# Geo3DSmart/PDANet

Measured on AMD Instinct MI355X. Metric: scenes/sec (16384-pt ONCE, PDA-SSD forward+backward), higher is better.
Workload: dtype f32; 1 GPU; once16k_b2_detector_fwd_bwd_adam; scenes_per_gpu=2, global_batch=2, parallelism=dp1, world_size_seen=1, cpu_affinity=GPU-local NUMA node of 0000:5d:00.0: 128 CPUs, full=False, graph_tail=False, graph_head=True

## Files before the change

include/pda_train.h:

```cpp
#ifndef PDA_TRAIN_H
#define PDA_TRAIN_H
#include "pda_pointnet2.h"

#ifdef __cplusplus
extern "C" {
#endif

int pda_grad_norm(const float *g, int64_t n, float *norm_out, float *scratch1024, pda_stream_t stream);
int pda_adam_onecycle_step(float *p, const float *g, float *m, float *v, int64_t n, float lr,
                           float beta1, float beta2, float eps, float wd, int step,
                           const float *total_norm, float max_norm, pda_stream_t stream);

int64_t pda_bn_relu_scratch_bytes(int c);
int pda_bn_relu_fwd(const float *x, const float *gamma, const float *beta, float *running_mean,
                    float *running_var, float *y, float *mean_invstd, void *scratch, int64_t rows, int c,
                    float eps, float momentum, pda_stream_t stream);
int pda_bn_relu_bwd(const float *x, const float *grad_y, const float *gamma, const float *beta,
                    const float *mean_invstd, float *grad_x, float *grad_gamma, float *grad_beta,
                    void *scratch, int64_t rows, int c, pda_stream_t stream);
int pda_bn_relu_fwd_counted(const float *x, const float *gamma, const float *beta, float *running_mean, float *running_var,
                            float *y, float *mean_invstd, void *scratch, int64_t rows, int c, float eps, float momentum,
                            const int32_t *count, int32_t *status, int relu, int training, pda_stream_t stream);
int pda_bn_relu_bwd_counted(const float *x, const float *grad_y, const float *gamma, const float *beta,
                            const float *mean_invstd, float *grad_x, float *grad_gamma, float *grad_beta, void *scratch,
// ... 38 lines not shown
                             float *grad_gamma, float *grad_beta, void *scratch, int64_t rows, int d,
                             pda_stream_t stream);

int64_t pda_linear_wgrad_scratch_bytes(int64_t tokens, int in_features, int out_features);
int pda_linear_wgrad_form(int64_t tokens, int in_features, int out_features);
int pda_linear_wgrad(const float *x, const float *grad_out, float *grad_weight, float *grad_bias,
                     void *scratch, int64_t tokens, int in_features, int out_features, pda_stream_t stream);
int pda_linear_wgrad_bn(const float *x, const float *grad_out, float *grad_weight, float *grad_bias, void *scratch,
                        int64_t tokens, int in_features, int out_features, const float *x_mean_invstd,
                        const float *x_gamma, const float *x_beta, pda_stream_t stream);

typedef struct pda_param_grad_entry {
    int32_t kind, count;
    const float *part, *part_bias;
    float *dst, *dst_bias;
    int64_t nm;
    int32_t n, cols;
    int64_t ld;
} pda_param_grad_entry_t;
int pda_linear_wgrad_partials(const float *x, const float *grad_out, void *scratch, int want_bias, int64_t tokens,
                              int in_features, int out_features, int *slices, pda_stream_t stream);
int pda_linear_wgrad_bn_partials(const float *x, const float *grad_out, void *scratch, int64_t tokens, int in_features,
                                 int out_features, const float *x_mean_invstd, const float *x_gamma,
                                 const float *x_beta, int *slices, pda_stream_t stream);
int pda_layer_norm_bwd_partials(const float *x, const float *grad_y, const void *grad_y2, int grad_y2_is_bf16,
                                const float *gamma, const float *mean_rstd, float *grad_x, uint16_t *grad_x_bf16,
                                void *scratch, int64_t rows, int d, int *nblocks, pda_stream_t stream);
int pda_param_grad_reduce_grouped(const pda_param_grad_entry_t *entries, int n, pda_stream_t stream);

int64_t pda_gemm_split_bn_tiles(int64_t tokens);
int pda_gemm_split_bn(const float *x, const void *wf, float *y, int64_t tokens, int k, int n_out,
                      const float *in_mean_invstd, const float *in_gamma, const float *in_beta, int stats_mode,
                      double *partial, pda_stream_t stream);
int pda_gemm_split_maxpool(const float *x, const void *wf, const float *bias, float *out, int64_t tokens, int k, int n_out,
                           int ns, int relu, pda_stream_t stream);
int pda_gemm_split_gather(const float *point_rows, const float *xyz, const float *new_xyz, const int32_t *idx,
                          const float *w1, int ldw1, const float *bias1, const void *wf, const float *bias2, float *y,
                          int b, int n, int m, int ns, int k, int n_out, int relu, pda_stream_t stream);
int pda_bn_stats_fwd(const float *x, float *running_mean, float *running_var, float *mean_invstd, void *scratch,
                     int64_t rows, int c, float eps, float momentum, pda_stream_t stream);
int pda_bn_finalize_fwd(const double *partial, int nblocks, int c, int64_t count, float eps, float momentum,
                        float *mean_invstd, float *running_mean, float *running_var, pda_stream_t stream);
int pda_bn_relu_max_pool_apply(const float *x, const float *gamma, const float *beta, const float *mean_invstd,
                               float *out, uint8_t *arg, int64_t groups, int ns, int c, pda_stream_t stream);

int64_t pda_colsum_scratch_bytes(int cols);
int pda_colsum_bf16(const uint16_t *g, float *out, void *scratch, int64_t rows, int cols, pda_stream_t stream);

int pda_assemble_tokens(const float *rppe, const float *dscale, const float *feats, const int32_t *idx,
                        const float *glob, float *out, int b, int n, int m, int nsample, int c,
                        pda_stream_t stream);
int pda_assemble_tokens_grad(const float *grad_out, const float *dscale, const float *feats, const int32_t *idx,
                             float *grad_rppe, float *grad_dscale, float *grad_feats, float *grad_glob,
                             int b, int n, int m, int nsample, int c, pda_stream_t stream);

int pda_add_max_pool(const float *a, const float *b, float *out, uint8_t *arg, int64_t groups, int seq, int d,
                     pda_stream_t stream);
int pda_max_pool_scatter(const float *grad_out, const uint8_t *arg, float *grad_x, int64_t groups, int seq,
                         int d, pda_stream_t stream);
int pda_add_max_pool_bf16(const float *a, const uint16_t *b, float *out, uint8_t *arg, int64_t groups, int seq,
                          int d, pda_stream_t stream);
int pda_max_pool_scatter_bf16(const float *grad_out, const uint8_t *arg, float *grad_x, uint16_t *grad_x_bf16,
                              int64_t groups, int seq, int d, pda_stream_t stream);

int pda_bn_relu_fwd_weighted(const float *x, const float *gamma, const float *beta, float *running_mean,
                             float *running_var, float *y, float *mean_invstd, void *scratch, int64_t rows, int c,
                             float eps, float momentum, const float *row_weight, int64_t count, pda_stream_t stream);
int pda_bn_relu_bwd_weighted(const float *x, const float *grad_y, const float *gamma, const float *beta,
                             const float *mean_invstd, float *grad_x, float *grad_gamma, float *grad_beta,
                             void *scratch, int64_t rows, int c, const float *row_weight, int64_t count,
                             pda_stream_t stream);

int pda_ragged_plan(const int32_t *idx, int32_t *cnt, int32_t *off, int32_t *rowmap, float *row_weight, int64_t groups,
                    int nsample, pda_stream_t stream);
int pda_assemble_tokens_ragged(const float *rppe, const float *dscale, const float *feats, const int32_t *idx,
                               const float *glob, const int32_t *rowmap, const int32_t *off, float *out,
                               int64_t max_tokens, int b, int n, int m, int nsample, int c, int rppe_compact,
                               pda_stream_t stream);
int pda_assemble_tokens_ragged_grad(const float *grad_out, const float *dscale, const float *feats,
                                    const int32_t *idx, const int32_t *cnt, const int32_t *off, const int32_t *rowmap,
                                    float *grad_rppe, float *grad_dscale, float *grad_feats, float *grad_glob,
                                    int64_t max_tokens, int b, int n, int m, int nsample, int c, int rppe_compact,
                                    pda_stream_t stream);
int pda_add_max_pool_ragged(const float *a, const float *b, const int32_t *cnt, const int32_t *off, float *out,
                            uint8_t *arg, int64_t groups, int d, pda_stream_t stream);
int pda_max_pool_scatter_ragged(const float *grad_out, const uint8_t *arg, const int32_t *rowmap,
                                const int32_t *off, float *grad_x, int64_t max_tokens, int64_t groups, int nsample,
                                int d, pda_stream_t stream);
int pda_group_attention_ragged_fwd(const float *qkv, const int32_t *cnt, const int32_t *off, float *out, float *lse,
                                   int64_t tokens, int64_t num_groups, int seq, int heads, int head_dim,
                                   pda_stream_t stream);
int pda_group_attention_ragged_bwd(const float *qkv, const float *grad_out, const float *lse, const int32_t *cnt,
                                   const int32_t *off, float *grad_qkv, int64_t tokens, int64_t num_groups, int seq,
                                   int heads, int head_dim, pda_stream_t stream);

int pda_densitynet_param_count(void);
int64_t pda_densitynet_scratch_bytes(void);
int pda_densitynet_fwd(const float *x, const float *params, float *y, float *stats, void *scratch,
                       float *running_mean1, float *running_var1, float *running_mean2, float *running_var2,
                       float *running_mean3, float *running_var3, int64_t n, float eps, float momentum,
                       pda_stream_t stream);
int pda_densitynet_bwd(const float *x, const float *grad_y, const float *params, const float *stats,
                       float *grad_params, void *scratch, int64_t n, float eps, pda_stream_t stream);
int pda_densitynet_fwd_unique(const float *x, const float *params, float *y, float *stats, void *scratch,
                              float *running_mean1, float *running_var1, float *running_mean2, float *running_var2,
                              float *running_mean3, float *running_var3, int64_t n, const int32_t *rowmap,
                              const float *row_weight, const int32_t *n_unique, int nsample, float eps, float momentum,
                              pda_stream_t stream);
int pda_densitynet_bwd_unique(const float *x, const float *grad_y, const float *params, const float *stats,
                              float *grad_params, void *scratch, int64_t n, const int32_t *rowmap,
                              const float *row_weight, const int32_t *n_unique, int nsample, float eps,
                              pda_stream_t stream);
#define PDA_DENSITYNET_MAX_SCALES 4
typedef struct pda_densitynet_scale {
    const float *x, *grad_y, *params;
    float *y, *stats;
    void *scratch;
    float *running[6];
    float *grad_params;
    int64_t n;
    const int32_t *rowmap;
    const float *row_weight;
    const int32_t *n_unique;
    int nsample;
    float eps, momentum;
} pda_densitynet_scale_t;
int pda_densitynet_fwd_multi(const pda_densitynet_scale_t *scales, int nscales, pda_stream_t stream);
int pda_densitynet_bwd_multi(const pda_densitynet_scale_t *scales, int nscales, pda_stream_t stream);

int pda_densitynet_eval_param_count(void);
int pda_densitynet_eval(const float *x, const float *folded, float *y, int64_t n, pda_stream_t stream);

int pda_pda_geometry(const float *xyz, const float *new_xyz, const int32_t *idx, float *rppe, float *dscale,
                     int b, int n, int m, int nsample, float radius, pda_stream_t stream);

int pda_points_in_boxes(const float *boxes, const float *pts, int32_t *box_idx_of_points, int b, int t,
                        int m, pda_stream_t stream);
int pda_roiaware_pool3d_fwd(const float *rois, const float *pts, const float *pts_feature, int32_t *argmax,
                            int32_t *pts_idx_of_voxels, float *pooled_features, int boxes_num, int pts_num,
                            int channels, int max_pts_each_voxel, int out_x, int out_y, int out_z, int pool_method,
                            pda_stream_t stream);
int pda_roiaware_pool3d_bwd(const int32_t *pts_idx_of_voxels, const int32_t *argmax, const float *grad_out,
                            float *grad_in, int boxes_num, int pts_num, int channels, int max_pts_each_voxel,
                            int out_x, int out_y, int out_z, int pool_method, pda_stream_t stream);
int pda_roipoint_pool3d_fwd(const float *xyz, const float *boxes3d, const float *pts_feature, float *pooled_features,
                            int32_t *pooled_empty_flag, int batch_size, int pts_num, int boxes_num, int channels,
                            int sampled_pts_num, pda_stream_t stream);
int pda_points_in_boxes_mask(const float *boxes, const float *pts, int32_t *mask, int boxes_num, int pts_num,
                             pda_stream_t stream);
int pda_points_in_boxes_count(const float *points, int stride, const float *boxes, int32_t *counts, int pts_num,
                              int batch_size, int boxes_num, pda_stream_t stream);
int pda_assign_point_targets(const float *gt_boxes, const int32_t *in_box, const int32_t *in_ext, int64_t *labels,
                             int64_t *box_idx, float *gt_of_points, int b, int n, int t, int mode, int single_class,
                             pda_stream_t stream);
int pda_head_assign_targets(const float *points, int point_stride, int point_offset, const float *gt_boxes, const float *extra_width,
                            int64_t *labels, int64_t *box_idx, float *gt_of_points, float *box_labels, const float *mean_size,
                            int bins, int b, int n, int t, int mode, int single_class, pda_stream_t stream);
int pda_sa_gaussian_mask(const float *coords, int stride, int offset, const float *gt_of_points, const int64_t *labels,
                         float *out, int64_t points, pda_stream_t stream);

int pda_boxes_overlap_bev(const float *boxes_a, const float *boxes_b, float *ans_overlap, int num_a,
                          int num_b, pda_stream_t stream);
int pda_boxes_iou_bev(const float *boxes_a, const float *boxes_b, float *ans_iou, int num_a, int num_b,
                      pda_stream_t stream);
int64_t pda_nms_mask_words(int n);
int pda_nms_bev(const float *boxes, const int32_t *num_valid, int64_t *keep, int32_t *num_keep,
// ... 335 lines not shown
```

pdanet_amd/_lib.py:

```python
import ctypes
import os

_HERE = os.path.dirname(os.path.abspath(__file__))
LIB_PATH = os.environ.get("PDA_LIB_PATH") or os.path.join(_HERE, "libpda_pointnet2.so")
ABI_VERSION = 20


class DensityNetScale(ctypes.Structure):
    _fields_ = [("x", ctypes.c_void_p), ("grad_y", ctypes.c_void_p), ("params", ctypes.c_void_p), ("y", ctypes.c_void_p),
                ("stats", ctypes.c_void_p), ("scratch", ctypes.c_void_p), ("running", ctypes.c_void_p * 6),
                ("grad_params", ctypes.c_void_p), ("n", ctypes.c_int64), ("rowmap", ctypes.c_void_p),
                ("row_weight", ctypes.c_void_p), ("n_unique", ctypes.c_void_p), ("nsample", ctypes.c_int),
                ("eps", ctypes.c_float), ("momentum", ctypes.c_float)]


class OnceFrames(ctypes.Structure):
    _fields_ = [("gt_boxes", ctypes.c_void_p), ("gt_name", ctypes.c_void_p), ("gt_offsets", ctypes.c_void_p),
                ("pred_boxes", ctypes.c_void_p), ("pred_score", ctypes.c_void_p), ("pred_name", ctypes.c_void_p),
                ("pred_start", ctypes.c_void_p), ("pred_count", ctypes.c_void_p), ("iou_start", ctypes.c_void_p),
                ("n_gt_total", ctypes.c_int64), ("pred_cap", ctypes.c_int64), ("iou_cap", ctypes.c_int64),
                ("n_frames", ctypes.c_int), ("max_gt", ctypes.c_int), ("max_pred", ctypes.c_int)]


class KittiFrames(ctypes.Structure):
# ... 16 lines not shown
_vp = ctypes.c_void_p
_i = ctypes.c_int
_f = ctypes.c_float

SIGNATURES = {
    "pda_furthest_point_sampling": [_vp, _vp, _vp, _i, _i, _i, _vp],
    "pda_furthest_point_sampling_with_dist": [_vp, _vp, _vp, _i, _i, _i, _vp],
    "pda_gather_points": [_vp, _vp, _vp, _i, _i, _i, _i, _vp],
    "pda_gather_points_grad": [_vp, _vp, _vp, _i, _i, _i, _i, _vp],
    "pda_ball_query": [_vp, _vp, _vp, _i, _i, _i, _f, _i, _vp],
    "pda_ball_query_dilated": [_vp, _vp, _vp, _i, _i, _i, _f, _f, _i, _vp],
    "pda_ellipsoid_query": [_vp, _vp, _vp, _i, _i, _i, _f, _f, _f, _i, _vp],
    "pda_ball_query_cells_scratch_bytes": [_i, _i],
    "pda_ball_query_cells": [_vp, _vp, ctypes.POINTER(_vp), _i, _i, _i, _i, ctypes.POINTER(_f), ctypes.POINTER(ctypes.c_int32),
                             _vp, ctypes.c_int64, _vp],
    "pda_ball_query_multi": [_vp, _vp, ctypes.POINTER(_vp), _i, _i, _i, _i,
                             ctypes.POINTER(_f), ctypes.POINTER(ctypes.c_int32), _vp],
    "pda_group_points": [_vp, _vp, _vp, _i, _i, _i, _i, _i, _vp],
    "pda_group_points_grad": [_vp, _vp, _vp, _i, _i, _i, _i, _i, _vp],
    "pda_group_rows": [_vp, _vp, _vp, _i, _i, _i, ctypes.c_int64, _vp],
    "pda_group_rows_grad": [_vp, _vp, _vp, _i, _i, _i, ctypes.c_int64, _vp],
    "pda_three_nn": [_vp, _vp, _vp, _vp, _i, _i, _i, _vp],
    "pda_three_interpolate": [_vp, _vp, _vp, _vp, _i, _i, _i, _i, _vp],
    "pda_three_interpolate_grad": [_vp, _vp, _vp, _vp, _i, _i, _i, _i, _vp],
    "pda_chamfer_forward": [_vp, _vp, _vp, _vp, _vp, _vp, _i, _i, _i, _vp],
    "pda_chamfer_backward": [_vp, _vp, _vp, _vp, _vp, _vp, _vp, _vp, _i, _i, _i, _vp],
    "pda_group_attention_fwd": [_vp, _vp, _vp, ctypes.c_int64, _i, _i, _i, _vp],
    "pda_group_attention_bwd": [_vp, _vp, _vp, _vp, ctypes.c_int64, _i, _i, _i, _vp],
    "pda_group_attention_fwd_bf16": [_vp, _vp, _vp, ctypes.c_int64, _i, _i, _i, _vp],
    "pda_group_attention_bwd_bf16": [_vp, _vp, _vp, _vp, ctypes.c_int64, _i, _i, _i, _vp],
    "pda_sa_mlp_maxpool": [_vp, _vp, _vp, _vp, _vp, _i, _i, _i, _i, _i, ctypes.POINTER(ctypes.c_int32),
                           ctypes.POINTER(_vp), ctypes.POINTER(_vp), ctypes.POINTER(_vp), _vp],
    "pda_linear_cols_packed_size": [_i, _i],
    "pda_linear_cols_pack": [_vp, _vp, _i, _i, _i, _i, _vp],
    "pda_linear_cols": [_vp, _vp, _vp, ctypes.c_int64, _i, _i, _vp],
    "pda_sa_gather_linear": [_vp, _vp, _vp, _vp, _vp, _vp, _i, _i, _i, _i, _i, _i, _vp],
    "pda_linear_split_packed_bytes": [_i, _i],
    "pda_linear_split_pack": [_vp, _vp, _i, _i, _i, _vp],
    "pda_linear_split_pack_both": [_vp, _vp, _vp, _i, _i, _vp],
    "pda_linear_split": [_vp, _vp, _vp, _vp, ctypes.c_int64, _i, _i, _i, _vp],
    "pda_gemm_split": [_vp, _vp, _vp, _vp, ctypes.c_int64, _i, _i, _i, _i, _vp],
    "pda_sa_mlp_packed_size": [_i, _i, _i],
    "pda_sa_mlp_pack_weights": [_vp, _vp, _i, _i, _i, _vp],
    "pda_grad_norm": [_vp, ctypes.c_int64, _vp, _vp, _vp],
    "pda_bn_relu_scratch_bytes": [_i],
    "pda_bn_relu_fwd": [_vp, _vp, _vp, _vp, _vp, _vp, _vp, _vp, ctypes.c_int64, _i, _f, _f, _vp],
    "pda_bn_relu_bwd": [_vp, _vp, _vp, _vp, _vp, _vp, _vp, _vp, _vp, ctypes.c_int64, _i, _vp],    "pda_bn_relu_fwd_mixed": [_vp, _i, _vp, _vp, _vp, _vp, _vp, _i, _vp, _vp, ctypes.c_int64, _i, _f, _f, _vp],
    "pda_bn_relu_bwd_mixed": [_vp, _i, _vp, _i, _vp, _vp, _vp, _vp, _vp, _vp, _vp, ctypes.c_int64, _i, _vp],
    "pda_bn_relu_max_pool_fwd": [_vp, _i, _vp, _vp, _vp, _vp, _vp, _vp, _vp, _vp, ctypes.c_int64, _i, _i, _f, _f, _vp],
    "pda_bn_relu_max_pool_bwd": [_vp, _i, _vp, _vp, _vp, _vp, _vp, _vp, _vp, _vp, _vp, ctypes.c_int64, _i, _i, _vp],

    "pda_layer_norm_scratch_bytes": [_i],
    "pda_layer_norm_fwd": [_vp, _vp, _vp, _vp, _vp, _vp, _vp, ctypes.c_int64, _i, _f, _vp],
    "pda_layer_norm_bwd": [_vp, _vp, _vp, _vp, _vp, _vp, _vp, _vp, _vp, ctypes.c_int64, _i, _vp],
    "pda_layer_norm_fwd_mixed": [_vp, _i, _vp, _vp, _vp, _vp, _vp, _vp, _vp, ctypes.c_int64, _i, _f, _vp],
    "pda_layer_norm_bwd_mixed": [_vp, _vp, _vp, _i, _vp, _vp, _vp, _vp, _vp, _vp, _vp, ctypes.c_int64, _i, _vp],
    "pda_linear_wgrad_scratch_bytes": [ctypes.c_int64, _i, _i],
    "pda_linear_wgrad_form": [ctypes.c_int64, _i, _i],
    "pda_linear_wgrad": [_vp, _vp, _vp, _vp, _vp, ctypes.c_int64, _i, _i, _vp],
    "pda_linear_wgrad_bn": [_vp, _vp, _vp, _vp, _vp, ctypes.c_int64, _i, _i, _vp, _vp, _vp, _vp],
    "pda_linear_wgrad_partials": [_vp, _vp, _vp, _i, ctypes.c_int64, _i, _i, ctypes.POINTER(_i), _vp],
    "pda_linear_wgrad_bn_partials": [_vp, _vp, _vp, ctypes.c_int64, _i, _i, _vp, _vp, _vp, ctypes.POINTER(_i), _vp],
    "pda_layer_norm_bwd_partials": [_vp, _vp, _vp, _i, _vp, _vp, _vp, _vp, _vp, ctypes.c_int64, _i, ctypes.POINTER(_i), _vp],
    "pda_param_grad_reduce_grouped": [ctypes.POINTER(ParamGradEntry), _i, _vp],
    "pda_gemm_split_bn_tiles": [ctypes.c_int64],
    "pda_gemm_split_bn": [_vp, _vp, _vp, ctypes.c_int64, _i, _i, _vp, _vp, _vp, _i, _vp, _vp],
    "pda_gemm_split_maxpool": [_vp, _vp, _vp, _vp, ctypes.c_int64, _i, _i, _i, _i, _vp],
    "pda_gemm_split_gather": [_vp, _vp, _vp, _vp, _vp, _i, _vp, _vp, _vp, _vp, _i, _i, _i, _i, _i, _i, _i, _vp],
    "pda_bn_stats_fwd": [_vp, _vp, _vp, _vp, _vp, ctypes.c_int64, _i, _f, _f, _vp],
    "pda_bn_finalize_fwd": [_vp, _i, _i, ctypes.c_int64, _f, _f, _vp, _vp, _vp, _vp],
    "pda_bn_relu_max_pool_apply": [_vp, _vp, _vp, _vp, _vp, _vp, ctypes.c_int64, _i, _i, _vp],
    "pda_bn_relu_bwd_reduce": [_vp, _vp, _vp, _vp, _vp, _vp, _vp, _vp, _vp, ctypes.c_int64, _i, _vp],
    "pda_colsum_scratch_bytes": [_i],
    "pda_colsum_bf16": [_vp, _vp, _vp, ctypes.c_int64, _i, _vp],
    "pda_assemble_tokens": [_vp, _vp, _vp, _vp, _vp, _vp, _i, _i, _i, _i, _i, _vp],
    "pda_assemble_tokens_grad": [_vp, _vp, _vp, _vp, _vp, _vp, _vp, _vp, _i, _i, _i, _i, _i, _vp],
    "pda_add_max_pool": [_vp, _vp, _vp, _vp, ctypes.c_int64, _i, _i, _vp],
    "pda_max_pool_scatter": [_vp, _vp, _vp, ctypes.c_int64, _i, _i, _vp],
    "pda_add_max_pool_bf16": [_vp, _vp, _vp, _vp, ctypes.c_int64, _i, _i, _vp],
    "pda_max_pool_scatter_bf16": [_vp, _vp, _vp, _vp, ctypes.c_int64, _i, _i, _vp],
    "pda_ragged_plan": [_vp, _vp, _vp, _vp, _vp, ctypes.c_int64, _i, _vp],
    "pda_assemble_tokens_ragged": [_vp, _vp, _vp, _vp, _vp, _vp, _vp, _vp, ctypes.c_int64, _i, _i, _i, _i, _i, _i, _vp],
    "pda_assemble_tokens_ragged_grad": [_vp, _vp, _vp, _vp, _vp, _vp, _vp, _vp, _vp, _vp, _vp, ctypes.c_int64, _i, _i, _i, _i, _i, _i, _vp],
    "pda_bn_relu_fwd_weighted": [_vp, _vp, _vp, _vp, _vp, _vp, _vp, _vp, ctypes.c_int64, _i, _f, _f, _vp, ctypes.c_int64, _vp],
    "pda_bn_relu_bwd_weighted": [_vp, _vp, _vp, _vp, _vp, _vp, _vp, _vp, _vp, ctypes.c_int64, _i, _vp, ctypes.c_int64, _vp],
    "pda_add_max_pool_ragged": [_vp, _vp, _vp, _vp, _vp, _vp, ctypes.c_int64, _i, _vp],
    "pda_max_pool_scatter_ragged": [_vp, _vp, _vp, _vp, _vp, ctypes.c_int64, ctypes.c_int64, _i, _i, _vp],
    "pda_group_attention_ragged_fwd": [_vp, _vp, _vp, _vp, _vp, ctypes.c_int64, ctypes.c_int64, _i, _i, _i, _vp],
    "pda_group_attention_ragged_bwd": [_vp, _vp, _vp, _vp, _vp, _vp, ctypes.c_int64, ctypes.c_int64, _i, _i, _i, _vp],
    "pda_densitynet_param_count": [],
    "pda_densitynet_eval_param_count": [],
    "pda_densitynet_scratch_bytes": [],
    "pda_densitynet_fwd": [_vp, _vp, _vp, _vp, _vp, _vp, _vp, _vp, _vp, _vp, _vp, ctypes.c_int64, _f, _f, _vp],
    "pda_densitynet_bwd": [_vp, _vp, _vp, _vp, _vp, _vp, ctypes.c_int64, _f, _vp],
    "pda_densitynet_eval": [_vp, _vp, _vp, ctypes.c_int64, _vp],
    "pda_densitynet_fwd_multi": [_vp, _i, _vp],
    "pda_densitynet_bwd_multi": [_vp, _i, _vp],
    "pda_densitynet_fwd_unique": [_vp, _vp, _vp, _vp, _vp, _vp, _vp, _vp, _vp, _vp, _vp, ctypes.c_int64, _vp, _vp, _vp, _i, _f, _f, _vp],
    "pda_densitynet_bwd_unique": [_vp, _vp, _vp, _vp, _vp, _vp, ctypes.c_int64, _vp, _vp, _vp, _i, _f, _vp],
    "pda_pda_geometry": [_vp, _vp, _vp, _vp, _vp, _i, _i, _i, _i, _f, _vp],
    "pda_points_in_boxes": [_vp, _vp, _vp, _i, _i, _i, _vp],
    "pda_roiaware_pool3d_fwd": [_vp, _vp, _vp, _vp, _vp, _vp, _i, _i, _i, _i, _i, _i, _i, _i, _vp],
    "pda_roiaware_pool3d_bwd": [_vp, _vp, _vp, _vp, _i, _i, _i, _i, _i, _i, _i, _i, _vp],
    "pda_roipoint_pool3d_fwd": [_vp, _vp, _vp, _vp, _vp, _i, _i, _i, _i, _i, _vp],
    "pda_points_in_boxes_mask": [_vp, _vp, _vp, _i, _i, _vp],
    "pda_points_in_boxes_count": [_vp, _i, _vp, _vp, _i, _i, _i, _vp],
    "pda_assign_point_targets": [_vp, _vp, _vp, _vp, _vp, _vp, _i, _i, _i, _i, _i, _vp],
    "pda_sa_gaussian_mask": [_vp, _i, _i, _vp, _vp, _vp, ctypes.c_int64, _vp],
    "pda_head_assign_targets": [_vp, _i, _i, _vp, ctypes.POINTER(ctypes.c_float), _vp, _vp, _vp, _vp, _vp, _i, _i, _i, _i, _i, _i, _vp],
    "pda_head_cls_loss": [_vp, _i, _i, _i, _vp, _vp, ctypes.c_int64, _f, _vp, _vp, _vp],
    "pda_head_centerness": [_vp, _vp, _vp, _vp, ctypes.c_int64, _vp],
    "pda_head_box_loss": [_vp, _vp, _vp, _vp, _f, _i, _f, _f, ctypes.c_int64, _vp, _vp, _vp],
    "pda_head_vote_loss": [_i, _vp, _vp, _vp, _vp, _i, _i, _i, _f, ctypes.c_int64, _vp, _vp, _vp],
    "pda_head_corner_loss": [_vp, _vp, _vp, _i, _vp, _vp, _vp, _i, _f, ctypes.c_int64, _vp, _vp, _vp, _vp],
    "pda_boxes_overlap_bev": [_vp, _vp, _vp, _i, _i, _vp],
    "pda_boxes_iou_bev": [_vp, _vp, _vp, _i, _i, _vp],
    "pda_nms_mask_words": [_i],
    "pda_nms_bev": [_vp, _vp, _vp, _vp, _vp, _i, _i, _f, _i, _vp],
    "pda_sa_small_train_workspace_bytes": [],
    "pda_sa_small_train_supported": [_i, _i, _i, _i, _i, ctypes.c_int64],
    "pda_sa_small_train_fwd": [_vp] * 7 + [ctypes.POINTER(_vp)] * 4 + [ctypes.POINTER(_f)] * 2 + [_vp] * 4 + [_i] * 8 + [_vp],
    "pda_sa_small_train_bwd": [_vp] * 13 + [ctypes.POINTER(_vp)] * 2 + [_i] * 8 + [_vp],
    "pda_sa_xyz_grad_scratch_bytes": [_i],
    "pda_sa_point_gather": [_vp, _vp, _vp, _vp, _vp, _i, _vp, _i, _vp, _i, _i, _i, _i, _i, _vp],
    "pda_sa_xyz_grad": [_vp, _vp, _vp, _vp, _vp, _i, _vp, _i, _vp, _vp, _i, _i, _i, _i, _i, _vp],
    "pda_sa_point_gather_stats_blocks": [ctypes.c_int64, _i],
    "pda_sa_point_gather_stats": [_vp, _vp, _vp, _vp, _vp, _i, _vp, _vp, _i, _i, _i, _i, _i, _vp],
    "pda_sa_point_grad_bn": [_vp] * 10 + [_i, _vp, _i, _vp, _vp, _vp, _i, _i, _i, _i, _i, _vp],
    "pda_adam_onecycle_step": [_vp, _vp, _vp, _vp, ctypes.c_int64, _f, _f, _f, _f, _f, _i, _vp, _f, _vp],
    "pda_input_stage_workspace_bytes": [_i, ctypes.c_int64],
    "pda_input_stage": [_vp, _vp, ctypes.c_int64, _i, _i, ctypes.c_int64, ctypes.POINTER(_f), _i, _vp, _vp, _vp,
                        ctypes.c_uint64, _i, _vp, _vp, _vp, _vp],
    "pda_input_boxes": [_vp, _vp, ctypes.c_int64, _i, _i, _i, ctypes.POINTER(_f), _i, _vp, _vp, _vp],
    "pda_augment_workspace_bytes": [_i, ctypes.c_int64, _i],
    "pda_augment": [_vp, _vp, ctypes.c_int64, _i, _i, ctypes.c_int64, _vp, _vp, ctypes.c_int64, _vp, _vp, ctypes.c_int64, _vp,
                    _vp, _vp, _i, _vp, _vp, _vp, _i, _vp, _vp, _vp, ctypes.POINTER(_f), ctypes.c_int64, _vp, ctypes.c_int64,
                    _vp, _vp, ctypes.c_int64, _vp, _vp, _vp, _vp],
    "pda_augment_paste": [_vp, _vp, ctypes.c_int64, _i, _i, ctypes.c_int64, _vp, _vp, ctypes.c_int64, _vp, _vp, ctypes.c_int64, _vp,
                          _vp, _vp, _i, _vp, _vp, _vp, _i, ctypes.POINTER(_f), ctypes.c_int64, _vp, ctypes.c_int64, _vp, _vp,
                          ctypes.c_int64, _vp, _vp, _vp, _vp],
    "pda_augment_steps_workspace_bytes": [_i, ctypes.c_int64, _i, _i],
    "pda_augment_steps": [_vp, _vp, ctypes.c_int64, _i, _i, ctypes.c_int64, _vp, _vp, ctypes.c_int64,
                          ctypes.POINTER(ctypes.c_int32), _i, _vp, _vp, _i, _i, _vp, _vp, ctypes.c_int64, _vp, _vp,
                          ctypes.c_int64, _vp, _vp, _vp, _vp],
    "pda_pyramid_aug_workspace_bytes": [_i, ctypes.c_int64, _i],
    "pda_pyramid_aug": [_vp, _vp, ctypes.c_int64, _i, _i, ctypes.c_int64, _vp, _vp, ctypes.c_int64, _vp, _vp, _vp, _vp, _vp, _i,
                        ctypes.POINTER(ctypes.c_double), _i, _i, _i, _vp, _vp, ctypes.c_int64, _vp, _vp, ctypes.c_int64, _vp,
                        _vp, _vp, _vp],
    "pda_once_eval_workspace_bytes": [_i, ctypes.c_int64, _i],
    "pda_once_eval_iou": [ctypes.POINTER(OnceFrames), _i, _vp, _vp, _vp],
    "pda_once_eval_accumulate": [ctypes.POINTER(OnceFrames), _vp, _vp, _i, _i, ctypes.POINTER(ctypes.c_double), _i, _vp, _vp,
                                 _vp, _vp],
    "pda_once_eval_match": [ctypes.POINTER(OnceFrames), _vp, _vp, _i, _i, ctypes.POINTER(ctypes.c_double), _i, _i, _vp, _vp,
                            _vp, _vp, _vp, _vp, _vp, _vp],
    "pda_kitti_eval_workspace_bytes": [_i, ctypes.c_int64, ctypes.c_int64, _i],
    "pda_kitti_eval_overlaps": [ctypes.POINTER(KittiFrames), _vp, _vp, _vp],
    "pda_kitti_eval_first_pass": [ctypes.POINTER(KittiFrames), _vp, _i, _i, _vp, _vp, _vp, ctypes.POINTER(ctypes.c_double),
                                  _vp, _vp, _vp, _vp, _vp, _vp],
    "pda_kitti_eval_match": [ctypes.POINTER(KittiFrames), _vp, _i, _i, _vp, _vp, _vp, ctypes.POINTER(ctypes.c_double), _i,
                             _vp, _vp, _vp, _vp, _vp, _vp, _vp, _vp, _vp, _vp, _vp],
    "pda_kitti_eval_predictions": [_vp, ctypes.c_int64, _i, _i, _vp, _vp, _vp, _i, _vp, _vp, _vp, _vp, _vp],
    "pda_recall_record": [_vp, _vp, _vp, _i, ctypes.POINTER(_f), _i, _vp, _vp, _i, _i, _i, _vp],
    "pda_roi_max_iou": [_vp, _vp, _vp, _i, _i, _vp, _vp, _i, _i, _i, _vp],
    "pda_roi_sample_targets": [_vp, _vp, _vp, _vp, _i, _vp, _vp, _i, _i] + [ctypes.c_double] * 5 + [_i, _vp, _vp, _vp, _vp,
                               ctypes.c_uint64] + [_vp] * 10 + [_i, _i, _i, _vp],
    "pda_kitti_fov_filter_workspace_bytes": [_i, ctypes.c_int64],
# ... 155 lines not shown
```

pdanet_amd/csrc/bn_relu.hip:

```cpp
#include "pda_common.h"

namespace pda {

constexpr int BN_BLOCKS = 512;

struct BnShape {
    int64_t rows;
    int c, cg, rpb;
    int ns;
    const float* roww;
    int64_t count;
};

__device__ __forceinline__ float4 pooled_grad(const float* __restrict__ gout, const uint8_t* __restrict__ arg, int64_t r,
                                              int col, const BnShape& s) {
    const int64_t g = r / s.ns;
    const int t = (int)(r - g * s.ns);
    const float4 v = reinterpret_cast<const float4*>(gout)[g * s.cg + col];
    const uchar4 k = reinterpret_cast<const uchar4*>(arg)[g * s.cg + col];
    return make_float4(k.x == t ? v.x : 0.f, k.y == t ? v.y : 0.f, k.z == t ? v.z : 0.f, k.w == t ? v.w : 0.f);
}

__device__ __forceinline__ void block_reduce_cols(double (&a)[4], double (&b)[4], double* lds, int cg, int rpb, double* out_a,
                                                  double* out_b) {
    const int tid = threadIdx.x;
    double* la = lds;
    double* lb = lds + 256 * 4;
#pragma unroll
    for (int k = 0; k < 4; ++k) { la[tid * 4 + k] = a[k]; lb[tid * 4 + k] = b[k]; }
    __syncthreads();
    if (tid < cg) {
        double sa[4] = {0, 0, 0, 0}, sb[4] = {0, 0, 0, 0};
        for (int r = 0; r < rpb; ++r)
#pragma unroll
            for (int k = 0; k < 4; ++k) { sa[k] += la[(r * cg + tid) * 4 + k]; sb[k] += lb[(r * cg + tid) * 4 + k]; }
#pragma unroll
        for (int k = 0; k < 4; ++k) { out_a[tid * 4 + k] = sa[k]; out_b[tid * 4 + k] = sb[k]; }
    }
}

template <bool BWD, typename TX, typename TD, bool POOL = false>
__global__ __launch_bounds__(256) void bn_reduce_kernel(const TX* __restrict__ x, const TD* __restrict__ dy,
                                                        const float* __restrict__ mean_invstd, const float* __restrict__ gamma,
                                                        const float* __restrict__ beta, double* __restrict__ partial, BnShape s,
                                                        const uint8_t* __restrict__ arg = nullptr) {
    __shared__ double lds[2 * 256 * 4];
    const int tid = threadIdx.x;
    double a[4] = {0, 0, 0, 0}, b[4] = {0, 0, 0, 0};
    if (s.cg <= 256) {
        const int col = tid % s.cg, r0 = tid / s.cg;
        float4 mu = make_float4(0, 0, 0, 0), is = mu, g = mu, be = mu;
        if (BWD) {
            mu = reinterpret_cast<const float4*>(mean_invstd)[col];
            is = reinterpret_cast<const float4*>(mean_invstd + s.c)[col];
            g = reinterpret_cast<const float4*>(gamma)[col];
            be = reinterpret_cast<const float4*>(beta)[col];
        }
        const int64_t stride = (int64_t)gridDim.x * s.rpb;
        auto row = [&](int64_t r, const float4& v, const float4& d) {
            if (!BWD) {
                const double w = s.roww ? (double)s.roww[r] : 1.0;
                a[0] += w * v.x; a[1] += w * v.y; a[2] += w * v.z; a[3] += w * v.w;
                b[0] += w * ((double)v.x * v.x); b[1] += w * ((double)v.y * v.y); b[2] += w * ((double)v.z * v.z); b[3] += w * ((double)v.w * v.w);
            } else {
                const float xh[4] = {(v.x - mu.x) * is.x, (v.y - mu.y) * is.y, (v.z - mu.z) * is.z, (v.w - mu.w) * is.w};
                const float gg[4] = {g.x, g.y, g.z, g.w}, bb[4] = {be.x, be.y, be.z, be.w}, dd[4] = {d.x, d.y, d.z, d.w};
#pragma unroll
                for (int k = 0; k < 4; ++k) {
                    const float dyh = (xh[k] * gg[k] + bb[k] > 0.f) ? dd[k] : 0.f;
                    a[k] += dyh;
                    b[k] += (double)dyh * xh[k];
                }
            }
        };
        auto grad = [&](int64_t r) -> float4 {
            if constexpr (!BWD) return make_float4(0, 0, 0, 0);
            else if constexpr (POOL) return pooled_grad(reinterpret_cast<const float*>(dy), arg, r, col, s);
            else return load4(dy + r * s.c + 4 * col);
        };
        constexpr int U = BWD ? 1 : 4;
        int64_t r = (int64_t)blockIdx.x * s.rpb + r0;
        for (; r + (U - 1) * stride < s.rows; r += U * stride) {
            float4 v[U], d[U];
#pragma unroll
            for (int u = 0; u < U; ++u) { v[u] = load4(x + (r + u * stride) * s.c + 4 * col); d[u] = grad(r + u * stride); }
#pragma unroll
            for (int u = 0; u < U; ++u) row(r + u * stride, v[u], d[u]);
        }
        for (; r < s.rows; r += stride) row(r, load4(x + r * s.c + 4 * col), grad(r));
    }
    double* pa = partial + (size_t)blockIdx.x * 2 * s.c;
    block_reduce_cols(a, b, lds, s.cg, s.rpb, pa, pa + s.c);
}

__device__ __forceinline__ bool sum_partials(const double* __restrict__ partial, int nblocks, int c, double& s1, double& s2, int& ch) {
    __shared__ double red[2][16][32];
    const int cl = threadIdx.x & 31, part = threadIdx.x >> 5;
    ch = blockIdx.x * 32 + cl;
    double a = 0, b = 0;
    if (ch < c) {
        double va[16], vb[16];
        for (int k0 = part; k0 < nblocks; k0 += 16 * 16) {
#pragma unroll
            for (int u = 0; u < 16; ++u) {
                const int k = k0 + 16 * u;
                va[u] = k < nblocks ? partial[(size_t)k * 2 * c + ch] : 0.0;
                vb[u] = k < nblocks ? partial[(size_t)k * 2 * c + c + ch] : 0.0;
            }
#pragma unroll
            for (int u = 0; u < 16; ++u) { a += va[u]; b += vb[u]; }
        }
    }
    red[0][part][cl] = a; red[1][part][cl] = b;
    __syncthreads();
    if (part != 0 || ch >= c) return false;
    s1 = 0; s2 = 0;
#pragma unroll
    for (int p = 0; p < 16; ++p) { s1 += red[0][p][cl]; s2 += red[1][p][cl]; }
    return true;
}

__global__ __launch_bounds__(512) void bn_finalize_fwd_kernel(const double* __restrict__ partial, int nblocks, int c, int64_t rows,
                                                               float eps, float momentum, float* __restrict__ mean_invstd,
                                                               float* __restrict__ running_mean, float* __restrict__ running_var) {
    double s1, s2;
    int ch;
    if (!sum_partials(partial, nblocks, c, s1, s2, ch)) return;
    const double mean = s1 / (double)rows;
    double var = s2 / (double)rows - mean * mean;
    var = var < 0 ? 0 : var;
    mean_invstd[ch] = (float)mean;
    mean_invstd[c + ch] = (float)(1.0 / sqrt(var + (double)eps));
    if (running_mean) {
        const double unbiased = rows > 1 ? var * ((double)rows / (double)(rows - 1)) : var;
        running_mean[ch] = (float)((1.0 - momentum) * running_mean[ch] + momentum * mean);
        running_var[ch] = (float)((1.0 - momentum) * running_var[ch] + momentum * unbiased);
    }
}

__global__ __launch_bounds__(512) void bn_finalize_bwd_kernel(const double* __restrict__ partial, int nblocks, int c, int64_t rows,
                                                               float* __restrict__ dgamma, float* __restrict__ dbeta,
                                                               float* __restrict__ sums) {
    double s1, s2;
    int ch;
    if (!sum_partials(partial, nblocks, c, s1, s2, ch)) return;
    dbeta[ch] = (float)s1;
    dgamma[ch] = (float)s2;
    sums[ch] = (float)(s1 / (double)rows);
    sums[c + ch] = (float)(s2 / (double)rows);
}

template <bool BWD, typename TX, typename TD, typename TO, bool POOL = false>
__global__ __launch_bounds__(256) void bn_apply_kernel(const TX* __restrict__ x, const TD* __restrict__ dy,
                                                       const float* __restrict__ mean_invstd, const float* __restrict__ gamma,
                                                       const float* __restrict__ beta, const float* __restrict__ sums,
                                                       TO* __restrict__ out, BnShape s, const uint8_t* __restrict__ arg = nullptr) {
    const int tid = threadIdx.x;
    const int col = tid % s.cg, r0 = tid / s.cg;
    const float4 mu = reinterpret_cast<const float4*>(mean_invstd)[col], is = reinterpret_cast<const float4*>(mean_invstd + s.c)[col];
    const float4 g = reinterpret_cast<const float4*>(gamma)[col], be = reinterpret_cast<const float4*>(beta)[col];
    float4 m1 = make_float4(0, 0, 0, 0), m2 = m1;
    if (BWD) { m1 = reinterpret_cast<const float4*>(sums)[col]; m2 = reinterpret_cast<const float4*>(sums + s.c)[col]; }
    const float muv[4] = {mu.x, mu.y, mu.z, mu.w}, isv[4] = {is.x, is.y, is.z, is.w}, gv[4] = {g.x, g.y, g.z, g.w},
                bv[4] = {be.x, be.y, be.z, be.w}, m1v[4] = {m1.x, m1.y, m1.z, m1.w}, m2v[4] = {m2.x, m2.y, m2.z, m2.w};
    const int64_t stride = (int64_t)gridDim.x * s.rpb;
    auto row = [&](int64_t r, const float4& v, const float4& d) {
        const float xv[4] = {v.x, v.y, v.z, v.w};
        float o[4];
        if (!BWD) {
#pragma unroll
            for (int k = 0; k < 4; ++k) o[k] = fmaxf((xv[k] - muv[k]) * isv[k] * gv[k] + bv[k], 0.f);
        } else {
            const float dv[4] = {d.x, d.y, d.z, d.w};
            const float w = s.roww ? s.roww[r] : 1.f;
#pragma unroll
            for (int k = 0; k < 4; ++k) {
                const float xh = (xv[k] - muv[k]) * isv[k];
// ... 67 lines not shown
    const int64_t cc = c > 0 ? c : 0;
    return (int64_t)pda::BN_BLOCKS * 2 * cc * (int64_t)sizeof(double) + 2 * cc * (int64_t)sizeof(float);
}

namespace pda {

template <typename T> static bool bn_aligned(const T* p) { return ((uintptr_t)p & (4 * sizeof(T) - 1)) == 0; }

template <typename TX, typename TY>
static int launch_bn_relu_fwd(const TX* x, const float* gamma, const float* beta, float* running_mean, float* running_var, TY* y,
                              float* mean_invstd, void* scratch, int64_t rows, int c, float eps, float momentum, hipStream_t st,
                              const char* what, const float* roww = nullptr, int64_t count = 0) {
    BnShape s;
    if (int rc = bn_shape(rows, c, s, what)) return rc;
    if (roww) { PDA_REQUIRE(count >= rows, "%s: count = %lld < rows", what, (long long)count); s.roww = roww; s.count = count; }
    PDA_REQUIRE(x && gamma && beta && y && mean_invstd && scratch, "%s: null pointer", what);
    PDA_REQUIRE((running_mean == nullptr) == (running_var == nullptr), "%s: running_mean/var must come together", what);
    PDA_REQUIRE(bn_aligned(x) && bn_aligned(y) && (((uintptr_t)gamma | (uintptr_t)beta | (uintptr_t)mean_invstd) & 15) == 0,
                "%s: pointers must be 16-byte aligned (8 for bf16 tensors)", what);
    const int grid = bn_grid(s);
    hipLaunchKernelGGL((bn_reduce_kernel<false, TX, float>), dim3(grid), dim3(256), 0, st, x, (const float*)nullptr, (const float*)nullptr,
                       (const float*)nullptr, (const float*)nullptr, (double*)scratch, s);
    hipLaunchKernelGGL(bn_finalize_fwd_kernel, dim3(divup(c, 32)), dim3(512), 0, st, (const double*)scratch, grid, c, s.count, eps, momentum,
                       mean_invstd, running_mean, running_var);
    hipLaunchKernelGGL((bn_apply_kernel<false, TX, float, TY>), dim3(grid), dim3(256), 0, st, x, (const float*)nullptr, mean_invstd, gamma, beta,
                       (const float*)nullptr, y, s);
    return check_launch(what);
}

template <typename TX, typename TD>
static int launch_bn_relu_bwd(const TX* x, const TD* grad_y, const float* gamma, const float* beta, const float* mean_invstd, TX* grad_x,
                              float* grad_gamma, float* grad_beta, void* scratch, int64_t rows, int c, hipStream_t st, const char* what,
                              const float* roww = nullptr, int64_t count = 0) {
    BnShape s;
    if (int rc = bn_shape(rows, c, s, what)) return rc;
    if (roww) { PDA_REQUIRE(count >= rows, "%s: count = %lld < rows", what, (long long)count); s.roww = roww; s.count = count; }
    PDA_REQUIRE(x && grad_y && gamma && beta && mean_invstd && grad_x && grad_gamma && grad_beta && scratch, "%s: null pointer", what);
    PDA_REQUIRE(bn_aligned(x) && bn_aligned(grad_y) && bn_aligned(grad_x) && (((uintptr_t)gamma | (uintptr_t)beta | (uintptr_t)mean_invstd) & 15) == 0,
                "%s: pointers must be 16-byte aligned (8 for bf16 tensors)", what);
    const int grid = bn_grid(s);
    float* sums = reinterpret_cast<float*>(reinterpret_cast<double*>(scratch) + (size_t)BN_BLOCKS * 2 * c);
    hipLaunchKernelGGL((bn_reduce_kernel<true, TX, TD>), dim3(grid), dim3(256), 0, st, x, grad_y, mean_invstd, gamma, beta, (double*)scratch, s);
    hipLaunchKernelGGL(bn_finalize_bwd_kernel, dim3(divup(c, 32)), dim3(512), 0, st, (const double*)scratch, grid, c, s.count, grad_gamma, grad_beta,
                       sums);
    hipLaunchKernelGGL((bn_apply_kernel<true, TX, TD, TX>), dim3(grid), dim3(256), 0, st, x, grad_y, mean_invstd, gamma, beta, sums, grad_x, s);
    return check_launch(what);
}

template <typename TX>
static int launch_bn_relu_pool_fwd(const TX* x, const float* gamma, const float* beta, float* running_mean, float* running_var, float* out,
                                   uint8_t* arg, float* mean_invstd, void* scratch, int64_t groups, int ns, int c, float eps,
                                   float momentum, hipStream_t st, const char* what) {
    PDA_REQUIRE(groups >= 1 && ns >= 1 && ns <= 255, "%s: groups=%lld ns=%d (1..255)", what, (long long)groups, ns);
    BnShape s;
    if (int rc = bn_shape(groups * ns, c, s, what)) return rc;
    s.ns = ns;
    PDA_REQUIRE(x && gamma && beta && out && arg && mean_invstd && scratch, "%s: null pointer", what);
    PDA_REQUIRE((running_mean == nullptr) == (running_var == nullptr), "%s: running_mean/var must come together", what);
    PDA_REQUIRE(bn_aligned(x) && (((uintptr_t)out | (uintptr_t)gamma | (uintptr_t)beta | (uintptr_t)mean_invstd) & 15) == 0 &&
                    ((uintptr_t)arg & 3) == 0, "%s: alignment", what);
    const int grid = bn_grid(s);
    hipLaunchKernelGGL((bn_reduce_kernel<false, TX, float>), dim3(grid), dim3(256), 0, st, x, (const float*)nullptr, (const float*)nullptr,
                       (const float*)nullptr, (const float*)nullptr, (double*)scratch, s, (const uint8_t*)nullptr);
    hipLaunchKernelGGL(bn_finalize_fwd_kernel, dim3(divup(c, 32)), dim3(512), 0, st, (const double*)scratch, grid, c, s.rows, eps, momentum,
                       mean_invstd, running_mean, running_var);
    hipLaunchKernelGGL(bn_apply_pool_kernel<TX>, dim3((unsigned)divup64(groups * s.cg, 256)), dim3(256), 0, st, x, mean_invstd, gamma, beta, out,
                       arg, groups, s);
    return check_launch(what);
}

template <typename TX>
static int launch_bn_relu_pool_bwd(const TX* x, const float* grad_out, const uint8_t* arg, const float* gamma, const float* beta,
                                   const float* mean_invstd, TX* grad_x, float* grad_gamma, float* grad_beta, void* scratch, int64_t groups,
                                   int ns, int c, hipStream_t st, const char* what) {
    PDA_REQUIRE(groups >= 1 && ns >= 1 && ns <= 255, "%s: groups=%lld ns=%d (1..255)", what, (long long)groups, ns);
    BnShape s;
    if (int rc = bn_shape(groups * ns, c, s, what)) return rc;
    s.ns = ns;
    PDA_REQUIRE(x && grad_out && arg && gamma && beta && mean_invstd && grad_x && grad_gamma && grad_beta && scratch, "%s: null pointer", what);
    PDA_REQUIRE(bn_aligned(x) && bn_aligned(grad_x) && (((uintptr_t)grad_out | (uintptr_t)gamma | (uintptr_t)beta | (uintptr_t)mean_invstd) & 15) == 0 &&
                    ((uintptr_t)arg & 3) == 0, "%s: alignment", what);
    const int grid = bn_grid(s);
    float* sums = reinterpret_cast<float*>(reinterpret_cast<double*>(scratch) + (size_t)BN_BLOCKS * 2 * c);
    hipLaunchKernelGGL((bn_reduce_kernel<true, TX, float, true>), dim3(grid), dim3(256), 0, st, x, grad_out, mean_invstd, gamma, beta,
                       (double*)scratch, s, arg);
    hipLaunchKernelGGL(bn_finalize_bwd_kernel, dim3(divup(c, 32)), dim3(512), 0, st, (const double*)scratch, grid, c, s.rows, grad_gamma, grad_beta,
                       sums);
    hipLaunchKernelGGL((bn_apply_kernel<true, TX, float, TX, true>), dim3(grid), dim3(256), 0, st, x, grad_out, mean_invstd, gamma, beta, sums,
                       grad_x, s, arg);
    return check_launch(what);
}


constexpr int BN_FLAG_FEW_ROWS = 8;

__device__ __forceinline__ int64_t bn_live_rows(const int32_t* __restrict__ count, int64_t rows) {
    const int32_t v = *count;
    return v < 0 ? 0 : (v > rows ? rows : (int64_t)v);
}

template <bool BWD, bool ADD = false>
__global__ __launch_bounds__(256) void bn_reduce_counted_kernel(const float* __restrict__ x, const float* __restrict__ dy,
                                                                const float* __restrict__ mean_invstd,
                                                                const float* __restrict__ gamma, const float* __restrict__ beta,
                                                                double* __restrict__ partial, BnShape s,
                                                                const int32_t* __restrict__ count, int relu,
                                                                const float* __restrict__ yout = nullptr) {
    static_assert(BWD || !ADD, "the forward statistics of the residual tail are those of the plain form");
    __shared__ double lds[2 * 256 * 4];
    const int tid = threadIdx.x;
    const int64_t n = bn_live_rows(count, s.rows);
    double a[4] = {0, 0, 0, 0}, b[4] = {0, 0, 0, 0};
    const int col = tid % s.cg, r0 = tid / s.cg;
    float4 mu = make_float4(0, 0, 0, 0), is = mu, g = mu, be = mu;
    if (BWD) {
        mu = reinterpret_cast<const float4*>(mean_invstd)[col];
        is = reinterpret_cast<const float4*>(mean_invstd + s.c)[col];
        g = reinterpret_cast<const float4*>(gamma)[col];
        be = reinterpret_cast<const float4*>(beta)[col];
    }
    const int64_t stride = (int64_t)gridDim.x * s.rpb;
    auto row = [&](const float4& v, const float4& d, const float4& yo) {
        if (!BWD) {
            a[0] += v.x; a[1] += v.y; a[2] += v.z; a[3] += v.w;
            b[0] += (double)v.x * v.x; b[1] += (double)v.y * v.y; b[2] += (double)v.z * v.z; b[3] += (double)v.w * v.w;
        } else {
            const float xh[4] = {(v.x - mu.x) * is.x, (v.y - mu.y) * is.y, (v.z - mu.z) * is.z, (v.w - mu.w) * is.w};
            const float gg[4] = {g.x, g.y, g.z, g.w}, bb[4] = {be.x, be.y, be.z, be.w}, dd[4] = {d.x, d.y, d.z, d.w};
            const float yy[4] = {yo.x, yo.y, yo.z, yo.w};
#pragma unroll
            for (int k = 0; k < 4; ++k) {
                const float dyh = (ADD ? yy[k] > 0.f : (!relu || xh[k] * gg[k] + bb[k] > 0.f)) ? dd[k] : 0.f;
                a[k] += dyh;
                b[k] += (double)dyh * xh[k];
            }
        }
    };
    auto saved = [&](int64_t r) -> float4 {
        if constexpr (ADD) return load4(yout + r * s.c + 4 * col);
        else return make_float4(0, 0, 0, 0);
    };
    constexpr int U = BWD ? 1 : 4;
    int64_t r = (int64_t)blockIdx.x * s.rpb + r0;
    for (; r + (U - 1) * stride < n; r += U * stride) {
        float4 v[U], d[U], yo[U];
#pragma unroll
        for (int u = 0; u < U; ++u) {
            v[u] = load4(x + (r + u * stride) * s.c + 4 * col);
            d[u] = BWD ? load4(dy + (r + u * stride) * s.c + 4 * col) : make_float4(0, 0, 0, 0);
            yo[u] = saved(r + u * stride);
        }
#pragma unroll
        for (int u = 0; u < U; ++u) row(v[u], d[u], yo[u]);
    }
    for (; r < n; r += stride)
        row(load4(x + r * s.c + 4 * col), BWD ? load4(dy + r * s.c + 4 * col) : make_float4(0, 0, 0, 0), saved(r));
    double* pa = partial + (size_t)blockIdx.x * 2 * s.c;
    block_reduce_cols(a, b, lds, s.cg, s.rpb, pa, pa + s.c);
}

__global__ __launch_bounds__(512) void bn_finalize_fwd_counted_kernel(const double* __restrict__ partial, int nblocks, int c,
                                                                       int64_t cap, const int32_t* __restrict__ count, float eps,
                                                                       float momentum, float* __restrict__ mean_invstd,
                                                                       float* __restrict__ running_mean,
                                                                       float* __restrict__ running_var, int32_t* __restrict__ status) {
    double s1, s2;
    int ch;
    const int64_t rows = bn_live_rows(count, cap);
    if (blockIdx.x == 0 && threadIdx.x == 0 && rows < 2) atomicOr(status, BN_FLAG_FEW_ROWS);
// ... 350 lines not shown
```

pdanet_amd/csrc/layer_norm.hip:

```cpp
#include "pda_common.h"
#include "param_grad_reduce.h"

namespace pda {

constexpr int LN_BLOCKS = 1024;

__device__ __forceinline__ float wave_sum(float v) {
#pragma unroll
    for (int o = 32; o >= 1; o >>= 1) v += __shfl_xor(v, o);
    return v;
}

template <int V, bool RESIDUAL, typename TX>
__global__ __launch_bounds__(256) void layer_norm_fwd_kernel(const TX* __restrict__ x, const float* __restrict__ res,
                                                             const float* __restrict__ gamma, const float* __restrict__ beta,
                                                             float* __restrict__ sum_out, float* __restrict__ y,
                                                             bf16_t* __restrict__ yb, float* __restrict__ mean_rstd, int64_t rows,
                                                             float eps) {
    constexpr int D = 256 * V;
    const int lane = lane_id();
    float4 g[V], be[V];
#pragma unroll
    for (int v = 0; v < V; ++v) {
        g[v] = reinterpret_cast<const float4*>(gamma)[v * 64 + lane];
        be[v] = reinterpret_cast<const float4*>(beta)[v * 64 + lane];
    }
    for (int64_t r = (int64_t)blockIdx.x * 4 + wave_id(); r < rows; r += (int64_t)gridDim.x * 4) {
        float4 a[V];
        float s = 0.f;
#pragma unroll
        for (int v = 0; v < V; ++v) {
            a[v] = load4(x + r * D + 4 * (v * 64 + lane));
            if (RESIDUAL) {
                const float4 b = reinterpret_cast<const float4*>(res + r * D)[v * 64 + lane];
                a[v].x += b.x; a[v].y += b.y; a[v].z += b.z; a[v].w += b.w;
                reinterpret_cast<float4*>(sum_out + r * D)[v * 64 + lane] = a[v];
            }
            s += (a[v].x + a[v].y) + (a[v].z + a[v].w);
        }
        const float mean = wave_sum(s) * (1.0f / D);
        float q = 0.f;
#pragma unroll
        for (int v = 0; v < V; ++v) {
            const float dx = a[v].x - mean, dy = a[v].y - mean, dz = a[v].z - mean, dw = a[v].w - mean;
            q += (dx * dx + dy * dy) + (dz * dz + dw * dw);
        }
        const float rstd = 1.0f / sqrtf(wave_sum(q) * (1.0f / D) + eps);
#pragma unroll
        for (int v = 0; v < V; ++v) {
            float4 o;
            o.x = (a[v].x - mean) * rstd * g[v].x + be[v].x;
            o.y = (a[v].y - mean) * rstd * g[v].y + be[v].y;
            o.z = (a[v].z - mean) * rstd * g[v].z + be[v].z;
            o.w = (a[v].w - mean) * rstd * g[v].w + be[v].w;
            if (y) reinterpret_cast<float4*>(y + r * D)[v * 64 + lane] = o;
            if (yb) store4(yb + r * D + 4 * (v * 64 + lane), o);
        }
        if (lane == 0) { mean_rstd[r * 2] = mean; mean_rstd[r * 2 + 1] = rstd; }
    }
}

template <int V, bool TWO, typename T2>
__global__ __launch_bounds__(256) void layer_norm_bwd_kernel(const float* __restrict__ x, const float* __restrict__ dy,
                                                             const T2* __restrict__ dy2, const float* __restrict__ gamma,
                                                             const float* __restrict__ mean_rstd, float* __restrict__ dx,
                                                             bf16_t* __restrict__ dxb, float* __restrict__ partial, int64_t rows) {
    constexpr int D = 256 * V;
    __shared__ float red[2][4][D];
    const int lane = lane_id(), w = wave_id();
    float4 g[V], sb[V], sg[V];
#pragma unroll
    for (int v = 0; v < V; ++v) {
        g[v] = reinterpret_cast<const float4*>(gamma)[v * 64 + lane];
        sb[v] = make_float4(0, 0, 0, 0); sg[v] = make_float4(0, 0, 0, 0);
    }
    for (int64_t r = (int64_t)blockIdx.x * 4 + w; r < rows; r += (int64_t)gridDim.x * 4) {
        const float mean = mean_rstd[r * 2], rstd = mean_rstd[r * 2 + 1];
        float4 xh[V], d[V];
        float s1 = 0.f, s2 = 0.f;
#pragma unroll
        for (int v = 0; v < V; ++v) {
            const float4 xv = reinterpret_cast<const float4*>(x + r * D)[v * 64 + lane];
            d[v] = reinterpret_cast<const float4*>(dy + r * D)[v * 64 + lane];
            if (TWO) {
                const float4 e = load4(dy2 + r * D + 4 * (v * 64 + lane));
                d[v].x += e.x; d[v].y += e.y; d[v].z += e.z; d[v].w += e.w;
            }
            xh[v] = make_float4((xv.x - mean) * rstd, (xv.y - mean) * rstd, (xv.z - mean) * rstd, (xv.w - mean) * rstd);
            sb[v].x += d[v].x; sb[v].y += d[v].y; sb[v].z += d[v].z; sb[v].w += d[v].w;
            sg[v].x += d[v].x * xh[v].x; sg[v].y += d[v].y * xh[v].y; sg[v].z += d[v].z * xh[v].z; sg[v].w += d[v].w * xh[v].w;
            d[v].x *= g[v].x; d[v].y *= g[v].y; d[v].z *= g[v].z; d[v].w *= g[v].w;
            s1 += (d[v].x + d[v].y) + (d[v].z + d[v].w);
            s2 += (d[v].x * xh[v].x + d[v].y * xh[v].y) + (d[v].z * xh[v].z + d[v].w * xh[v].w);
        }
        const float m1 = wave_sum(s1) * (1.0f / D), m2 = wave_sum(s2) * (1.0f / D);
#pragma unroll
        for (int v = 0; v < V; ++v) {
            float4 o;
            o.x = rstd * (d[v].x - m1 - xh[v].x * m2);
            o.y = rstd * (d[v].y - m1 - xh[v].y * m2);
            o.z = rstd * (d[v].z - m1 - xh[v].z * m2);
            o.w = rstd * (d[v].w - m1 - xh[v].w * m2);
            reinterpret_cast<float4*>(dx + r * D)[v * 64 + lane] = o;
            if (dxb) store4(dxb + r * D + 4 * (v * 64 + lane), o);
        }
    }
#pragma unroll
    for (int v = 0; v < V; ++v) {
        reinterpret_cast<float4*>(red[0][w])[v * 64 + lane] = sb[v];
        reinterpret_cast<float4*>(red[1][w])[v * 64 + lane] = sg[v];
    }
    __syncthreads();
    for (int c = threadIdx.x; c < D; c += 256) {
        partial[((size_t)blockIdx.x * 2 + 0) * D + c] = (red[0][0][c] + red[0][1][c]) + (red[0][2][c] + red[0][3][c]);
        partial[((size_t)blockIdx.x * 2 + 1) * D + c] = (red[1][0][c] + red[1][1][c]) + (red[1][2][c] + red[1][3][c]);
    }
}

__global__ __launch_bounds__(1024) void layer_norm_finalize_kernel(const float* __restrict__ partial, int nblocks, int d,
                                                                   float* __restrict__ dgamma, float* __restrict__ dbeta) {
    __shared__ float red[2][16][64];
    layer_norm_finalize_block(partial, nblocks, d, dgamma, dbeta, (int)blockIdx.x, red);
}

static int ln_grid(int64_t rows) {
    const int64_t b = divup64(rows, 4);
    return (int)(b < LN_BLOCKS ? b : LN_BLOCKS);
}

}

PDA_API int64_t pda_layer_norm_scratch_bytes(int d) { return (int64_t)pda::LN_BLOCKS * 2 * (d > 0 ? d : 0) * (int64_t)sizeof(float); }

namespace pda {

template <typename TX>
static int launch_layer_norm_fwd(const TX* x, const float* residual, const float* gamma, const float* beta, float* sum_out, float* y,
                                 bf16_t* yb, float* mean_rstd, int64_t rows, int d, float eps, hipStream_t st, const char* what) {
    PDA_REQUIRE(rows >= 0, "%s: rows = %lld", what, (long long)rows);
    PDA_REQUIRE(d == 256 || d == 512 || d == 1024, "%s: D = %d (256, 512 or 1024)", what, d);
    if (rows == 0) return PDA_OK;
    PDA_REQUIRE(x && gamma && beta && (y || yb) && mean_rstd, "%s: null pointer", what);
    PDA_REQUIRE((residual == nullptr) == (sum_out == nullptr), "%s: residual and sum_out come together", what);
    PDA_REQUIRE((((uintptr_t)y | (uintptr_t)gamma | (uintptr_t)beta | (uintptr_t)residual | (uintptr_t)sum_out) & 15) == 0 &&
                    (((uintptr_t)x | (uintptr_t)yb) & (4 * sizeof(TX) - 1) & 15) == 0 && ((uintptr_t)yb & 7) == 0,
                "%s: pointers must be 16-byte aligned (8 for bf16 tensors)", what);
    const dim3 grid(ln_grid(rows)), block(256);
#define PDA_LN_FWD(V)                                                                                                          \
    if (residual) hipLaunchKernelGGL((layer_norm_fwd_kernel<V, true, TX>), grid, block, 0, st, x, residual, gamma, beta, sum_out, y, yb, mean_rstd, rows, eps); \
    else hipLaunchKernelGGL((layer_norm_fwd_kernel<V, false, TX>), grid, block, 0, st, x, residual, gamma, beta, sum_out, y, yb, mean_rstd, rows, eps)
    if (d == 256) { PDA_LN_FWD(1); } else if (d == 512) { PDA_LN_FWD(2); } else { PDA_LN_FWD(4); }
#undef PDA_LN_FWD
    return check_launch(what);
}

template <typename T2>
static int launch_layer_norm_bwd(const float* x, const float* grad_y, const T2* grad_y2, const float* gamma, const float* mean_rstd,
                                 float* grad_x, bf16_t* grad_x_b, float* grad_gamma, float* grad_beta, void* scratch, int64_t rows, int d,
                                 hipStream_t st, const char* what, int* nblocks_out = nullptr) {
    PDA_REQUIRE(rows >= 1, "%s: rows = %lld", what, (long long)rows);
    PDA_REQUIRE(d == 256 || d == 512 || d == 1024, "%s: D = %d (256, 512 or 1024)", what, d);
    PDA_REQUIRE(x && grad_y && gamma && mean_rstd && grad_x && ((grad_gamma && grad_beta) || nblocks_out) && scratch, "%s: null pointer", what);
    PDA_REQUIRE((((uintptr_t)x | (uintptr_t)grad_y | (uintptr_t)grad_x | (uintptr_t)gamma) & 15) == 0 &&
                    ((uintptr_t)grad_y2 & (4 * sizeof(T2) - 1)) == 0 && ((uintptr_t)grad_x_b & 7) == 0,
                "%s: pointers must be 16-byte aligned (8 for bf16 tensors)", what);
    const int nblocks = ln_grid(rows);
    const dim3 grid(nblocks), block(256);
    float* partial = (float*)scratch;
#define PDA_LN_BWD(V)                                                                                                               \
    if (grad_y2) hipLaunchKernelGGL((layer_norm_bwd_kernel<V, true, T2>), grid, block, 0, st, x, grad_y, grad_y2, gamma, mean_rstd, grad_x, grad_x_b, partial, rows); \
    else hipLaunchKernelGGL((layer_norm_bwd_kernel<V, false, T2>), grid, block, 0, st, x, grad_y, grad_y2, gamma, mean_rstd, grad_x, grad_x_b, partial, rows)
    if (d == 256) { PDA_LN_BWD(1); } else if (d == 512) { PDA_LN_BWD(2); } else { PDA_LN_BWD(4); }
#undef PDA_LN_BWD
    if (nblocks_out) *nblocks_out = nblocks;
    else hipLaunchKernelGGL(layer_norm_finalize_kernel, dim3(divup(d, 64)), dim3(1024), 0, st, partial, nblocks, d, grad_gamma, grad_beta);
    return check_launch(what);
}

}

PDA_API int pda_layer_norm_fwd(const float* x, const float* residual, const float* gamma, const float* beta, float* sum_out,
                               float* y, float* mean_rstd, int64_t rows, int d, float eps, pda_stream_t stream) {
    PDA_REQUIRE(y != nullptr || rows == 0, "pda_layer_norm_fwd: null pointer");
    return pda::launch_layer_norm_fwd<float>(x, residual, gamma, beta, sum_out, y, nullptr, mean_rstd, rows, d, eps, (hipStream_t)stream,
                                             "pda_layer_norm_fwd");
}

PDA_API int pda_layer_norm_fwd_mixed(const void* x, int x_is_bf16, const float* residual, const float* gamma, const float* beta,
                                     float* sum_out, float* y, uint16_t* y_bf16, float* mean_rstd, int64_t rows, int d, float eps,
                                     pda_stream_t stream) {
    if (x_is_bf16)
        return pda::launch_layer_norm_fwd<pda::bf16_t>((const pda::bf16_t*)x, residual, gamma, beta, sum_out, y, y_bf16, mean_rstd, rows, d,
                                                       eps, (hipStream_t)stream, "pda_layer_norm_fwd_mixed");
    return pda::launch_layer_norm_fwd<float>((const float*)x, residual, gamma, beta, sum_out, y, y_bf16, mean_rstd, rows, d, eps,
                                             (hipStream_t)stream, "pda_layer_norm_fwd_mixed");
}

PDA_API int pda_layer_norm_bwd(const float* x, const float* grad_y, const float* grad_y2, const float* gamma, const float* mean_rstd,
                               float* grad_x, float* grad_gamma, float* grad_beta, void* scratch, int64_t rows, int d,
                               pda_stream_t stream) {
    return pda::launch_layer_norm_bwd<float>(x, grad_y, grad_y2, gamma, mean_rstd, grad_x, nullptr, grad_gamma, grad_beta, scratch, rows, d,
                                             (hipStream_t)stream, "pda_layer_norm_bwd");
}

PDA_API int pda_layer_norm_bwd_mixed(const float* x, const float* grad_y, const void* grad_y2, int grad_y2_is_bf16, const float* gamma,
                                     const float* mean_rstd, float* grad_x, uint16_t* grad_x_bf16, float* grad_gamma, float* grad_beta,
                                     void* scratch, int64_t rows, int d, pda_stream_t stream) {
    if (grad_y2_is_bf16)
        return pda::launch_layer_norm_bwd<pda::bf16_t>(x, grad_y, (const pda::bf16_t*)grad_y2, gamma, mean_rstd, grad_x, grad_x_bf16,
                                                       grad_gamma, grad_beta, scratch, rows, d, (hipStream_t)stream, "pda_layer_norm_bwd_mixed");
// ... 111 lines not shown
```

pdanet_amd/csrc/ragged.hip:

```cpp
#include "pda_common.h"

namespace pda {

__global__ __launch_bounds__(256) void ragged_count_kernel(const int32_t* __restrict__ idx, int32_t* __restrict__ cnt, int groups, int ns) {
    const int g = blockIdx.x * 256 + threadIdx.x;
    if (g >= groups) return;
    const int32_t* row = idx + (size_t)g * ns;
    const int32_t first = row[0];
    int32_t c = 1;
    for (int s = 1; s < ns; ++s) c += row[s] != first ? 1 : 0;
    cnt[g] = c;
}

__global__ __launch_bounds__(1024) void ragged_plan_kernel(const int32_t* __restrict__ cnt, int32_t* __restrict__ off, int groups) {
    __shared__ int32_t part[1024];
    const int t = threadIdx.x;
    const int per = (groups + 1023) / 1024;
    const int g0 = t * per, g1 = min(groups, g0 + per);
    int32_t sum = 0;
    for (int g = g0; g < g1; ++g) sum += cnt[g];
    part[t] = sum;
    __syncthreads();
    for (int o = 1; o < 1024; o <<= 1) {
        const int32_t v = t >= o ? part[t - o] : 0;
        __syncthreads();
        part[t] += v;
        __syncthreads();
    }
    int32_t run = part[t] - sum;
    for (int g = g0; g < g1; ++g) { off[g] = run; run += cnt[g]; }
    if (t == 1023) off[groups] = part[1023];
}

__global__ __launch_bounds__(256) void ragged_rowmap_kernel(const int32_t* __restrict__ cnt, const int32_t* __restrict__ off,
                                                            int32_t* __restrict__ rowmap, float* __restrict__ roww, int64_t total,
                                                            int ns) {
    const int64_t e = (int64_t)blockIdx.x * 256 + threadIdx.x;
    if (e >= total) return;
    const int g = (int)(e / ns), s = (int)(e % ns);
    const int c = cnt[g];
    if (s < c) {
        rowmap[off[g] + s] = (int32_t)e;
        if (roww) roww[off[g] + s] = s == 0 ? (float)(ns - c + 1) : 1.f;
    }
}

__global__ __launch_bounds__(256) void assemble_ragged_fwd_kernel(const float* __restrict__ rppe, const float* __restrict__ dscale,
                                                                  const float* __restrict__ feats, const int* __restrict__ idx,
                                                                  const float* __restrict__ glob, const int32_t* __restrict__ rowmap,
                                                                  const int32_t* __restrict__ off, float* __restrict__ out, int n,
                                                                  int m, int ns, int c4, int groups, int rppe_compact) {
    const int64_t total = (int64_t)off[groups] * c4;
    const int64_t e = (int64_t)blockIdx.x * 256 + threadIdx.x;
    if (e >= total) return;
    const int c = (int)(e % c4);
    const int64_t u = e / c4;
    const int64_t tok = rowmap[u];
    const int64_t bm = tok / ns;
    const int64_t b = bm / m;
    const float4 r = reinterpret_cast<const float4*>(rppe)[(rppe_compact ? u : tok) * c4 + c];
    const float4 f = reinterpret_cast<const float4*>(feats)[((size_t)b * n + idx[tok]) * c4 + c];
    const float4 g = reinterpret_cast<const float4*>(glob)[bm * c4 + c];
    const float d = dscale[tok];
    float4* o = reinterpret_cast<float4*>(out) + (size_t)u * 4 * c4 + c;
    o[0] = r;
    o[c4] = make_float4(f.x * d, f.y * d, f.z * d, f.w * d);
    o[2 * c4] = f;
    o[3 * c4] = g;
}

template <int c4>
__global__ __launch_bounds__(256) void assemble_ragged_bwd_kernel(const float* __restrict__ dx, const float* __restrict__ dscale,
                                                                  const float* __restrict__ feats, const int* __restrict__ idx,
                                                                  const int32_t* __restrict__ cnt, const int32_t* __restrict__ off,
                                                                  float* __restrict__ d_rppe, float* __restrict__ d_dscale,
                                                                  float* __restrict__ d_feats, float* __restrict__ d_glob, int n,
                                                                  int m, int ns, int64_t total, int rppe_compact) {
    const int64_t e = (int64_t)blockIdx.x * 256 + threadIdx.x;
    const bool live = e < total;
    const int64_t ec = live ? e : total - 1;
    const int c = (int)(ec % c4);
    const int64_t bm = ec / c4;
    const int64_t b = bm / m;
    const int64_t tok0 = bm * ns;
    const int n_tok = cnt[bm];
    const int64_t u0 = off[bm];
    const float4* frows = reinterpret_cast<const float4*>(feats) + (size_t)b * n * c4 + c;
    float4 acc_g = make_float4(0.f, 0.f, 0.f, 0.f);
    const float4 zero = make_float4(0.f, 0.f, 0.f, 0.f);
    for (int t = 0; t < ns; ++t) {
        const int64_t tok = tok0 + t;
        if (t >= n_tok) {
            if (live) {
                if (!rppe_compact) reinterpret_cast<float4*>(d_rppe)[(size_t)tok * c4 + c] = zero;
                if (c == 0) d_dscale[tok] = 0.f;
            }
            continue;
        }
        const float4* g4 = reinterpret_cast<const float4*>(dx) + (size_t)(u0 + t) * 4 * c4 + c;
        const float4 g_r = g4[0], g_fd = g4[c4], g_f = g4[2 * c4], g_g = g4[3 * c4];
        const int row = idx[tok];
        const float4 f = frows[(size_t)row * c4];
        const float d = dscale[tok];
        float part = (g_fd.x * f.x + g_fd.y * f.y) + (g_fd.z * f.z + g_fd.w * f.w);
#pragma unroll
        for (int o = c4 >> 1; o >= 1; o >>= 1) part += __shfl_xor(part, o);
        acc_g.x += g_g.x; acc_g.y += g_g.y; acc_g.z += g_g.z; acc_g.w += g_g.w;
        if (live) {
            reinterpret_cast<float4*>(d_rppe)[(size_t)(rppe_compact ? u0 + t : tok) * c4 + c] = g_r;
            if (c == 0) d_dscale[tok] = part;
            float* df = d_feats + (((size_t)b * n + row) * c4 + c) * 4;
            atomicAdd(df + 0, g_fd.x * d + g_f.x); atomicAdd(df + 1, g_fd.y * d + g_f.y);
            atomicAdd(df + 2, g_fd.z * d + g_f.z); atomicAdd(df + 3, g_fd.w * d + g_f.w);
        }
    }
    if (live) reinterpret_cast<float4*>(d_glob)[bm * c4 + c] = acc_g;
}

template <int c4>
__global__ __launch_bounds__(256) void assemble_ragged_bwd_token_kernel(const float* __restrict__ dx, const float* __restrict__ dscale,
                                                                        const float* __restrict__ feats, const int* __restrict__ idx,
                                                                        const int32_t* __restrict__ rowmap, const int32_t* __restrict__ off,
                                                                        float* __restrict__ d_rppe, float* __restrict__ d_dscale,
                                                                        float* __restrict__ d_feats, int n, int m, int ns, int groups,
                                                                        int rppe_compact) {
    const int64_t total = (int64_t)off[groups] * c4;
    const int64_t e = (int64_t)blockIdx.x * 256 + threadIdx.x;
    const bool live = e < total;
    const int64_t ec = live ? e : (total > 0 ? total - 1 : 0);
    if (total == 0) return;
    const int c = (int)(ec % c4);
    const int64_t u = ec / c4;
    const int64_t tok = rowmap[u];
    const int64_t b = (tok / ns) / m;
    const float4* g4 = reinterpret_cast<const float4*>(dx) + (size_t)u * 4 * c4 + c;
    const float4 g_r = g4[0], g_fd = g4[c4], g_f = g4[2 * c4];
    const int row = idx[tok];
    const float4 f = (reinterpret_cast<const float4*>(feats) + (size_t)b * n * c4 + c)[(size_t)row * c4];
    const float d = dscale[tok];
    float part = (g_fd.x * f.x + g_fd.y * f.y) + (g_fd.z * f.z + g_fd.w * f.w);
#pragma unroll
    for (int o = c4 >> 1; o >= 1; o >>= 1) part += __shfl_xor(part, o);
    if (!live) return;
    reinterpret_cast<float4*>(d_rppe)[(size_t)(rppe_compact ? u : tok) * c4 + c] = g_r;
    if (c == 0) d_dscale[tok] = part;
    float* df = d_feats + (((size_t)b * n + row) * c4 + c) * 4;
    atomicAdd(df + 0, g_fd.x * d + g_f.x); atomicAdd(df + 1, g_fd.y * d + g_f.y);
    atomicAdd(df + 2, g_fd.z * d + g_f.z); atomicAdd(df + 3, g_fd.w * d + g_f.w);
}

__global__ __launch_bounds__(256) void assemble_ragged_bwd_group_kernel(const float* __restrict__ dx, const int32_t* __restrict__ cnt,
                                                                        const int32_t* __restrict__ off, float* __restrict__ d_rppe,
                                                                        float* __restrict__ d_dscale, float* __restrict__ d_glob, int c4,
                                                                        int ns, int64_t total, int rppe_compact) {
    const int64_t e = (int64_t)blockIdx.x * 256 + threadIdx.x;
    if (e >= total) return;
    const int c = (int)(e % c4);
    const int64_t bm = e / c4;
    const int n_tok = cnt[bm];
    const float4* g4 = reinterpret_cast<const float4*>(dx) + (size_t)off[bm] * 4 * c4 + 3 * c4 + c;
    float4 acc = make_float4(0.f, 0.f, 0.f, 0.f);
    int t = 0;
    for (; t + 4 <= n_tok; t += 4) {
        float4 v[4];
#pragma unroll
        for (int q = 0; q < 4; ++q) v[q] = g4[(size_t)(t + q) * 4 * c4];
#pragma unroll
        for (int q = 0; q < 4; ++q) { acc.x += v[q].x; acc.y += v[q].y; acc.z += v[q].z; acc.w += v[q].w; }
    }
    for (; t < n_tok; ++t) { const float4 v = g4[(size_t)t * 4 * c4]; acc.x += v.x; acc.y += v.y; acc.z += v.z; acc.w += v.w; }
    reinterpret_cast<float4*>(d_glob)[bm * c4 + c] = acc;
    const float4 zero = make_float4(0.f, 0.f, 0.f, 0.f);
    for (t = n_tok; t < ns; ++t) {
        if (!rppe_compact) reinterpret_cast<float4*>(d_rppe)[(size_t)(bm * ns + t) * c4 + c] = zero;
        if (c == 0) d_dscale[bm * ns + t] = 0.f;
    }
}

__global__ __launch_bounds__(256) void add_max_pool_ragged_kernel(const float* __restrict__ a, const float* __restrict__ b,
                                                                  const int32_t* __restrict__ cnt, const int32_t* __restrict__ off,
                                                                  float* __restrict__ out, uint8_t* __restrict__ arg, int64_t groups,
                                                                  int d4) {
    const int64_t e = (int64_t)blockIdx.x * 256 + threadIdx.x;
    if (e >= groups * d4) return;
    const int64_t g = e / d4;
    const int c = (int)(e % d4);
    const int s = cnt[g];
    const float4* pa = reinterpret_cast<const float4*>(a) + (size_t)off[g] * d4 + c;
    const float4* pb = reinterpret_cast<const float4*>(b) + (size_t)off[g] * d4 + c;
    float4 best = make_float4(-__builtin_inff(), -__builtin_inff(), -__builtin_inff(), -__builtin_inff());
    uchar4 bi = make_uchar4(0, 0, 0, 0);
    for (int t = 0; t < s; ++t) {
        const float4 x = pa[(size_t)t * d4], y = pb[(size_t)t * d4];
        const float4 v = make_float4(x.x + y.x, x.y + y.y, x.z + y.z, x.w + y.w);
        if (v.x > best.x) { best.x = v.x; bi.x = (uint8_t)t; }
        if (v.y > best.y) { best.y = v.y; bi.y = (uint8_t)t; }
        if (v.z > best.z) { best.z = v.z; bi.z = (uint8_t)t; }
        if (v.w > best.w) { best.w = v.w; bi.w = (uint8_t)t; }
    }
    reinterpret_cast<float4*>(out)[e] = best;
    reinterpret_cast<uchar4*>(arg)[e] = bi;
}

__global__ __launch_bounds__(256) void max_pool_scatter_ragged_kernel(const float* __restrict__ dout, const uint8_t* __restrict__ arg,
                                                                      const int32_t* __restrict__ rowmap, const int32_t* __restrict__ off,
                                                                      float* __restrict__ dx, int groups, int ns, int d4) {
    const int64_t total = (int64_t)off[groups] * d4;
    const int64_t e = (int64_t)blockIdx.x * 256 + threadIdx.x;
    if (e >= total) return;
    const int c = (int)(e % d4);
    const int64_t u = e / d4;
    const int32_t tok = rowmap[u];
    const int64_t g = tok / ns;
    const int t = tok % ns;
    const float4 v = reinterpret_cast<const float4*>(dout)[g * d4 + c];
    const uchar4 k = reinterpret_cast<const uchar4*>(arg)[g * d4 + c];
    reinterpret_cast<float4*>(dx)[e] = make_float4(k.x == t ? v.x : 0.f, k.y == t ? v.y : 0.f, k.z == t ? v.z : 0.f, k.w == t ? v.w : 0.f);
}

static bool ragged_c_ok(int c) { return c == 16 || c == 32 || c == 64 || c == 128 || c == 256; }

}

PDA_API int pda_ragged_plan(const int32_t* idx, int32_t* cnt, int32_t* off, int32_t* rowmap, float* row_weight, int64_t groups,
                            int nsample, pda_stream_t stream) {
    PDA_REQUIRE(groups >= 0 && groups <= (1 << 24) && nsample >= 1 && nsample <= 255 && groups * nsample < INT32_MAX,
                "pda_ragged_plan: groups=%lld nsample=%d", (long long)groups, nsample);
    PDA_REQUIRE(off != nullptr, "pda_ragged_plan: null pointer");
    PDA_REQUIRE(groups == 0 || (idx && cnt && rowmap), "pda_ragged_plan: null pointer");
    if (groups > 0)
        hipLaunchKernelGGL(pda::ragged_count_kernel, dim3((unsigned)pda::divup64(groups, 256)), dim3(256), 0, (hipStream_t)stream, idx, cnt,
                           (int)groups, nsample);
    hipLaunchKernelGGL(pda::ragged_plan_kernel, dim3(1), dim3(1024), 0, (hipStream_t)stream, cnt, off, (int)groups);
    if (groups > 0) {
        const int64_t total = groups * nsample;
        hipLaunchKernelGGL(pda::ragged_rowmap_kernel, dim3((unsigned)pda::divup64(total, 256)), dim3(256), 0, (hipStream_t)stream, cnt,
                           off, rowmap, row_weight, total, nsample);
    }
    return pda::check_launch("pda_ragged_plan");
}

PDA_API int pda_assemble_tokens_ragged(const float* rppe, const float* dscale, const float* feats, const int32_t* idx,
                                       const float* glob, const int32_t* rowmap, const int32_t* off, float* out, int64_t max_tokens,
                                       int b, int n, int m, int nsample, int c, int rppe_compact, pda_stream_t stream) {
    PDA_REQUIRE(b >= 0 && n >= 1 && m >= 0 && nsample >= 1 && max_tokens >= 0 && pda::ragged_c_ok(c),
                "pda_assemble_tokens_ragged: b=%d n=%d m=%d nsample=%d C=%d", b, n, m, nsample, c);
    const int64_t total = max_tokens * (c / 4);
    if (total == 0 || (int64_t)b * m == 0) return PDA_OK;
    PDA_REQUIRE(rppe && dscale && feats && idx && glob && rowmap && off && out, "pda_assemble_tokens_ragged: null pointer");
    PDA_REQUIRE((((uintptr_t)rppe | (uintptr_t)feats | (uintptr_t)glob | (uintptr_t)out) & 15) == 0, "pda_assemble_tokens_ragged: alignment");
    hipLaunchKernelGGL(pda::assemble_ragged_fwd_kernel, dim3((unsigned)pda::divup64(total, 256)), dim3(256), 0, (hipStream_t)stream, rppe,
                       dscale, feats, idx, glob, rowmap, off, out, n, m, nsample, c / 4, b * m, rppe_compact);
    return pda::check_launch("pda_assemble_tokens_ragged");
}

PDA_API int pda_assemble_tokens_ragged_grad(const float* grad_out, const float* dscale, const float* feats, const int32_t* idx,
                                            const int32_t* cnt, const int32_t* off, const int32_t* rowmap, float* grad_rppe,
                                            float* grad_dscale, float* grad_feats, float* grad_glob, int64_t max_tokens, int b, int n,
                                            int m, int nsample, int c, int rppe_compact, pda_stream_t stream) {
    PDA_REQUIRE(b >= 0 && n >= 1 && m >= 0 && nsample >= 1 && max_tokens >= 0 && pda::ragged_c_ok(c),
                "pda_assemble_tokens_ragged_grad: b=%d n=%d m=%d nsample=%d C=%d", b, n, m, nsample, c);
    const int64_t centre_cols = (int64_t)b * m * (c / 4);
    if (centre_cols == 0) return PDA_OK;
    PDA_REQUIRE(grad_out && dscale && feats && idx && cnt && off && grad_rppe && grad_dscale && grad_feats && grad_glob,
                "pda_assemble_tokens_ragged_grad: null pointer");
    PDA_REQUIRE((((uintptr_t)grad_out | (uintptr_t)feats | (uintptr_t)grad_rppe | (uintptr_t)grad_glob) & 15) == 0,
                "pda_assemble_tokens_ragged_grad: alignment");
    const dim3 grid((unsigned)pda::divup64(centre_cols, 256)), block(256);
    if (rowmap) {
        const int64_t tok_cols = max_tokens * (c / 4);
        if (tok_cols > 0) {
            const dim3 tgrid((unsigned)pda::divup64(tok_cols, 256));
#define PDA_ASM_TOK(C4)                                                                                                               \
    case C4: hipLaunchKernelGGL(pda::assemble_ragged_bwd_token_kernel<C4>, tgrid, block, 0, (hipStream_t)stream, grad_out, dscale, feats, \
                                idx, rowmap, off, grad_rppe, grad_dscale, grad_feats, n, m, nsample, b * m, rppe_compact); break
            switch (c / 4) { PDA_ASM_TOK(4); PDA_ASM_TOK(8); PDA_ASM_TOK(16); PDA_ASM_TOK(32); PDA_ASM_TOK(64); }
#undef PDA_ASM_TOK
        }
        hipLaunchKernelGGL(pda::assemble_ragged_bwd_group_kernel, grid, block, 0, (hipStream_t)stream, grad_out, cnt, off, grad_rppe,
                           grad_dscale, grad_glob, c / 4, nsample, centre_cols, rppe_compact);
        return pda::check_launch("pda_assemble_tokens_ragged_grad");
    }
#define PDA_ASM_BWD(C4)                                                                                                          \
    case C4: hipLaunchKernelGGL(pda::assemble_ragged_bwd_kernel<C4>, grid, block, 0, (hipStream_t)stream, grad_out, dscale, feats, idx, \
                                cnt, off, grad_rppe, grad_dscale, grad_feats, grad_glob, n, m, nsample, centre_cols, rppe_compact); break
    switch (c / 4) { PDA_ASM_BWD(4); PDA_ASM_BWD(8); PDA_ASM_BWD(16); PDA_ASM_BWD(32); PDA_ASM_BWD(64); }
#undef PDA_ASM_BWD
    return pda::check_launch("pda_assemble_tokens_ragged_grad");
}

PDA_API int pda_add_max_pool_ragged(const float* a, const float* b, const int32_t* cnt, const int32_t* off, float* out, uint8_t* arg,
                                    int64_t groups, int d, pda_stream_t stream) {
    PDA_REQUIRE(groups >= 0 && d >= 4 && (d & 3) == 0, "pda_add_max_pool_ragged: groups=%lld d=%d", (long long)groups, d);
    if (groups == 0) return PDA_OK;
    PDA_REQUIRE(a && b && cnt && off && out && arg, "pda_add_max_pool_ragged: null pointer");
    PDA_REQUIRE((((uintptr_t)a | (uintptr_t)b | (uintptr_t)out) & 15) == 0 && ((uintptr_t)arg & 3) == 0, "pda_add_max_pool_ragged: alignment");
    const int64_t n = groups * (d / 4);
    hipLaunchKernelGGL(pda::add_max_pool_ragged_kernel, dim3((unsigned)pda::divup64(n, 256)), dim3(256), 0, (hipStream_t)stream, a, b, cnt,
                       off, out, arg, groups, d / 4);
    return pda::check_launch("pda_add_max_pool_ragged");
}

PDA_API int pda_max_pool_scatter_ragged(const float* grad_out, const uint8_t* arg, const int32_t* rowmap, const int32_t* off,
                                        float* grad_x, int64_t max_tokens, int64_t groups, int nsample, int d, pda_stream_t stream) {
    PDA_REQUIRE(groups >= 0 && groups < INT32_MAX && max_tokens >= 0 && nsample >= 1 && d >= 4 && (d & 3) == 0,
                "pda_max_pool_scatter_ragged: groups=%lld d=%d", (long long)groups, d);
    if (groups == 0 || max_tokens == 0) return PDA_OK;
    PDA_REQUIRE(grad_out && arg && rowmap && off && grad_x, "pda_max_pool_scatter_ragged: null pointer");
    PDA_REQUIRE((((uintptr_t)grad_out | (uintptr_t)grad_x) & 15) == 0 && ((uintptr_t)arg & 3) == 0, "pda_max_pool_scatter_ragged: alignment");
    const int64_t n = max_tokens * (d / 4);
    hipLaunchKernelGGL(pda::max_pool_scatter_ragged_kernel, dim3((unsigned)pda::divup64(n, 256)), dim3(256), 0, (hipStream_t)stream,
                       grad_out, arg, rowmap, off, grad_x, (int)groups, nsample, d / 4);
    return pda::check_launch("pda_max_pool_scatter_ragged");
}
```

pdanet_amd/pointnet2_batch_cuda.py:

```python
import ctypes

import functools
import os
import threading

import torch

from . import _lib
from . import param_cache


def _chk(t, name, dtype):
    if not isinstance(t, torch.Tensor):
        raise TypeError("%s must be a torch.Tensor" % name)
    if not t.is_cuda:
        raise RuntimeError("%s must be a CUDA(HIP) tensor -- there is no CPU path" % name)
    if not t.is_contiguous():
        raise RuntimeError("%s must be contiguous" % name)
    if t.dtype != dtype:
        raise RuntimeError("%s must be %s, got %s" % (name, dtype, t.dtype))
    return t.data_ptr()


def _numel_ok(t, n, name):
# ... 662 lines not shown
    _numel_ok(grad_out, groups * d, "grad_out"); _numel_ok(arg, groups * d, "arg"); _numel_ok(grad_x, groups * seq * d, "grad_x")
    if grad_x_bf16 is not None:
        _numel_ok(grad_x_bf16, groups * seq * d, "grad_x_bf16")
        _call("pda_max_pool_scatter_bf16", grad_out, _chk(grad_out, "grad_out", F32), _chk(arg, "arg", torch.uint8), _chk(grad_x, "grad_x", F32),
              _chk(grad_x_bf16, "grad_x_bf16", BF16), groups, seq, d)
        return 1
    _call("pda_max_pool_scatter", grad_out, _chk(grad_out, "grad_out", F32), _chk(arg, "arg", torch.uint8), _chk(grad_x, "grad_x", F32),
          groups, seq, d)
    return 1


def assemble_tokens(rppe, dscale, feats, idx, glob, out, b, n, m, nsample, c):
    t = b * m * nsample
    _numel_ok(rppe, t * c, "rppe"); _numel_ok(dscale, t, "dscale"); _numel_ok(feats, b * n * c, "feats"); _numel_ok(idx, t, "idx")
    _numel_ok(glob, b * m * c, "glob"); _numel_ok(out, t * 4 * c, "out")
    _call("pda_assemble_tokens", rppe, _chk(rppe, "rppe", F32), _chk(dscale, "dscale", F32), _chk(feats, "feats", F32),
          _chk(idx, "idx", I32), _chk(glob, "glob", F32), _chk(out, "out", F32), b, n, m, nsample, c)
    return 1


def assemble_tokens_grad(grad_out, dscale, feats, idx, grad_rppe, grad_dscale, grad_feats, grad_glob, b, n, m, nsample, c):
    t = b * m * nsample
    _numel_ok(grad_out, t * 4 * c, "grad_out"); _numel_ok(grad_rppe, t * c, "grad_rppe"); _numel_ok(grad_dscale, t, "grad_dscale")
    _numel_ok(grad_feats, b * n * c, "grad_feats"); _numel_ok(grad_glob, b * m * c, "grad_glob")
    _call("pda_assemble_tokens_grad", grad_out, _chk(grad_out, "grad_out", F32), _chk(dscale, "dscale", F32), _chk(feats, "feats", F32),
          _chk(idx, "idx", I32), _chk(grad_rppe, "grad_rppe", F32), _chk(grad_dscale, "grad_dscale", F32),
          _chk(grad_feats, "grad_feats", F32), _chk(grad_glob, "grad_glob", F32), b, n, m, nsample, c)
    return 1


def ragged_plan(idx, cnt, off, rowmap, groups, nsample, roww=None):
    _numel_ok(idx, groups * nsample, "idx"); _numel_ok(cnt, groups, "cnt"); _numel_ok(off, groups + 1, "off")
    _numel_ok(rowmap, groups * nsample, "rowmap")
    if roww is not None:
        _numel_ok(roww, groups * nsample, "roww")
    _call("pda_ragged_plan", idx, _chk(idx, "idx", I32), _chk(cnt, "cnt", I32), _chk(off, "off", I32), _chk(rowmap, "rowmap", I32),
          None if roww is None else _chk(roww, "roww", F32), groups, nsample)
    return 1


def bn_relu_fwd_weighted(x, gamma, beta, running_mean, running_var, y, mean_invstd, scratch, rows, c, eps, momentum, roww, count):
    _numel_ok(x, rows * c, "x"); _numel_ok(y, rows * c, "y"); _numel_ok(mean_invstd, 2 * c, "mean_invstd"); _numel_ok(roww, rows, "roww")
    rm = None if running_mean is None else _chk(running_mean, "running_mean", F32)
    rv = None if running_var is None else _chk(running_var, "running_var", F32)
    _buffers_written(rm)
    _call("pda_bn_relu_fwd_weighted", x, _chk(x, "x", F32), _chk(gamma, "gamma", F32), _chk(beta, "beta", F32), rm, rv, _chk(y, "y", F32),
          _chk(mean_invstd, "mean_invstd", F32), _chk(scratch, "scratch", torch.uint8), rows, c, float(eps), float(momentum),
          _chk(roww, "roww", F32), int(count))
    return 1


def bn_relu_bwd_weighted(x, grad_y, gamma, beta, mean_invstd, grad_x, grad_gamma, grad_beta, scratch, rows, c, roww, count):
    _numel_ok(x, rows * c, "x"); _numel_ok(grad_y, rows * c, "grad_y"); _numel_ok(grad_x, rows * c, "grad_x"); _numel_ok(roww, rows, "roww")
    _call("pda_bn_relu_bwd_weighted", x, _chk(x, "x", F32), _chk(grad_y, "grad_y", F32), _chk(gamma, "gamma", F32), _chk(beta, "beta", F32),
          _chk(mean_invstd, "mean_invstd", F32), _chk(grad_x, "grad_x", F32), _chk(grad_gamma, "grad_gamma", F32),
          _chk(grad_beta, "grad_beta", F32), _chk(scratch, "scratch", torch.uint8), rows, c, _chk(roww, "roww", F32), int(count))
    return 1


def assemble_tokens_ragged(rppe, dscale, feats, idx, glob, rowmap, off, out, tokens, b, n, m, nsample, c, rppe_compact=False):
    t = b * m * nsample
    _numel_ok(rppe, (tokens if rppe_compact else t) * c, "rppe"); _numel_ok(dscale, t, "dscale"); _numel_ok(feats, b * n * c, "feats"); _numel_ok(idx, t, "idx")
    _numel_ok(glob, b * m * c, "glob"); _numel_ok(out, tokens * 4 * c, "out"); _numel_ok(rowmap, tokens, "rowmap"); _numel_ok(off, b * m + 1, "off")
    _call("pda_assemble_tokens_ragged", rppe, _chk(rppe, "rppe", F32), _chk(dscale, "dscale", F32), _chk(feats, "feats", F32),
          _chk(idx, "idx", I32), _chk(glob, "glob", F32), _chk(rowmap, "rowmap", I32), _chk(off, "off", I32), _chk(out, "out", F32),
          tokens, b, n, m, nsample, c, 1 if rppe_compact else 0)
    return 1


def assemble_tokens_ragged_grad(grad_out, dscale, feats, idx, cnt, off, grad_rppe, grad_dscale, grad_feats, grad_glob, tokens, b, n, m, nsample, c,
                                rppe_compact=False, rowmap=None):
    t = b * m * nsample
    if rowmap is not None:
        _numel_ok(rowmap, tokens, "rowmap")
    _numel_ok(grad_out, tokens * 4 * c, "grad_out"); _numel_ok(grad_rppe, (tokens if rppe_compact else t) * c, "grad_rppe"); _numel_ok(grad_dscale, t, "grad_dscale")
    _numel_ok(grad_feats, b * n * c, "grad_feats"); _numel_ok(grad_glob, b * m * c, "grad_glob"); _numel_ok(cnt, b * m, "cnt"); _numel_ok(off, b * m + 1, "off")
    _call("pda_assemble_tokens_ragged_grad", grad_out, _chk(grad_out, "grad_out", F32), _chk(dscale, "dscale", F32), _chk(feats, "feats", F32),
          _chk(idx, "idx", I32), _chk(cnt, "cnt", I32), _chk(off, "off", I32), None if rowmap is None else _chk(rowmap, "rowmap", I32),
          _chk(grad_rppe, "grad_rppe", F32), _chk(grad_dscale, "grad_dscale", F32), _chk(grad_feats, "grad_feats", F32),
          _chk(grad_glob, "grad_glob", F32), tokens, b, n, m, nsample, c, 1 if rppe_compact else 0)
    return 1


def add_max_pool_ragged(a, b, cnt, off, out, arg, tokens, groups, d):
    _numel_ok(a, tokens * d, "a"); _numel_ok(b, tokens * d, "b"); _numel_ok(out, groups * d, "out"); _numel_ok(arg, groups * d, "arg")
    _numel_ok(cnt, groups, "cnt"); _numel_ok(off, groups + 1, "off")
    _call("pda_add_max_pool_ragged", a, _chk(a, "a", F32), _chk(b, "b", F32), _chk(cnt, "cnt", I32), _chk(off, "off", I32),
          _chk(out, "out", F32), _chk(arg, "arg", torch.uint8), groups, d)
    return 1


def max_pool_scatter_ragged(grad_out, arg, rowmap, off, grad_x, tokens, groups, nsample, d):
    _numel_ok(grad_out, groups * d, "grad_out"); _numel_ok(arg, groups * d, "arg"); _numel_ok(grad_x, tokens * d, "grad_x")
    _numel_ok(rowmap, tokens, "rowmap"); _numel_ok(off, groups + 1, "off")
    _call("pda_max_pool_scatter_ragged", grad_out, _chk(grad_out, "grad_out", F32), _chk(arg, "arg", torch.uint8),
          _chk(rowmap, "rowmap", I32), _chk(off, "off", I32), _chk(grad_x, "grad_x", F32), tokens, groups, nsample, d)
    return 1


def group_attention_ragged_fwd(qkv, cnt, off, out, lse, tokens, num_groups, seq, heads, head_dim):
    _numel_ok(qkv, tokens * 3 * heads * head_dim, "qkv"); _numel_ok(out, tokens * heads * head_dim, "out")
    _numel_ok(lse, num_groups * heads * seq, "lse"); _numel_ok(cnt, num_groups, "cnt"); _numel_ok(off, num_groups + 1, "off")
    _call("pda_group_attention_ragged_fwd", qkv, _chk(qkv, "qkv", F32), _chk(cnt, "cnt", I32), _chk(off, "off", I32),
          _chk(out, "out", F32), _chk(lse, "lse", F32), tokens, num_groups, seq, heads, head_dim)
    return 1


def group_attention_ragged_bwd(qkv, grad_out, lse, cnt, off, grad_qkv, tokens, num_groups, seq, heads, head_dim):
    _numel_ok(qkv, tokens * 3 * heads * head_dim, "qkv"); _numel_ok(grad_qkv, tokens * 3 * heads * head_dim, "grad_qkv")
    _numel_ok(grad_out, tokens * heads * head_dim, "grad_out"); _numel_ok(lse, num_groups * heads * seq, "lse")
    _call("pda_group_attention_ragged_bwd", qkv, _chk(qkv, "qkv", F32), _chk(grad_out, "grad_out", F32), _chk(lse, "lse", F32),
          _chk(cnt, "cnt", I32), _chk(off, "off", I32), _chk(grad_qkv, "grad_qkv", F32), tokens, num_groups, seq, heads, head_dim)
    return 1


def linear_cols_pack(w, n_out, k, transposed_source=False, gather_order=False):
    lib = _lib.load()
    wf = torch.empty((_cols_packed_size(int(n_out), int(k)),), dtype=F32, device=w.device)
    _numel_ok(w, n_out * k, "w")
    _call("pda_linear_cols_pack", w, _chk(w, "w", F32), _chk(wf, "wf", F32), n_out, k, 1 if transposed_source else 0,
          1 if gather_order else 0)
    return wf


def linear_cols(x, wf, y, tokens, k, n_out):
    _numel_ok(x, tokens * k, "x"); _numel_ok(y, tokens * n_out, "y")
    _numel_ok(wf, _cols_packed_size(int(n_out), int(k)), "wf")
    _call("pda_linear_cols", x, _chk(x, "x", F32), _chk(wf, "wf", F32), _chk(y, "y", F32), tokens, k, n_out)
    return 1


def linear_split_pack(w, n_out, k, transposed_source=False):
    lib = _lib.load()
    wf = torch.empty((_split_packed_bytes(int(n_out), int(k)),), dtype=torch.uint8, device=w.device)
    _numel_ok(w, n_out * k, "w")
    _call("pda_linear_split_pack", w, _chk(w, "w", F32), _chk(wf, "wf", torch.uint8), n_out, k, 1 if transposed_source else 0)
    return wf


def linear_split_pack_both(w, n_out, k):
    wf = torch.empty((_split_packed_bytes(int(n_out), int(k)),), dtype=torch.uint8, device=w.device)
    wft = torch.empty((_split_packed_bytes(int(k), int(n_out)),), dtype=torch.uint8, device=w.device)
    _numel_ok(w, n_out * k, "w")
    _call("pda_linear_split_pack_both", w, _chk(w, "w", F32), _chk(wf, "wf", torch.uint8), _chk(wft, "wft", torch.uint8), n_out, k)
    return wf, wft


def linear_split(x, wf, bias, y, tokens, k, n_out, relu=False):
    _numel_ok(x, tokens * k, "x"); _numel_ok(y, tokens * n_out, "y")
    _numel_ok(wf, _split_packed_bytes(int(n_out), int(k)), "wf")
    if bias is not None:
        _numel_ok(bias, n_out, "bias")
    _call("pda_linear_split", x, _chk(x, "x", F32), _chk(wf, "wf", torch.uint8), None if bias is None else _chk(bias, "bias", F32),
          _chk(y, "y", F32), tokens, k, n_out, 1 if relu else 0)
    return 1


def gemm_split(x, wf, bias, y, tokens, k, n_out, relu=False, accumulate=False):
    _numel_ok(x, tokens * k, "x"); _numel_ok(y, tokens * n_out, "y")
    _numel_ok(wf, _split_packed_bytes(int(n_out), int(k)), "wf")
    if bias is not None:
        _numel_ok(bias, n_out, "bias")
    _call("pda_gemm_split", x, _chk(x, "x", F32), _chk(wf, "wf", torch.uint8), None if bias is None else _chk(bias, "bias", F32),
          _chk(y, "y", F32), tokens, k, n_out, 1 if relu else 0, 1 if accumulate else 0)
    return 1

# ... 116 lines not shown
```

pdanet_amd/pointnet2_modules.py:

```python
from typing import List

import os

import torch
import torch.nn as nn
import torch.nn.functional as F

from . import param_cache
from . import pointnet2_utils


class TransformerEncoderLayerPreNorm(nn.Module):

    def __init__(self, d_model, nhead, dim_feedforward=2048, dropout=0.1, activation="relu"):
        super().__init__()
        self.self_attn = nn.MultiheadAttention(d_model, nhead, dropout=dropout)
        self.linear1 = nn.Linear(d_model, dim_feedforward)
        self.dropout = nn.Dropout(dropout, inplace=True)
        self.linear2 = nn.Linear(dim_feedforward, d_model)
        self.norm1 = nn.LayerNorm(d_model)
        self.norm2 = nn.LayerNorm(d_model)
        self.dropout1 = nn.Dropout(dropout, inplace=True)
        self.dropout2 = nn.Dropout(dropout, inplace=True)
        self.activation = nn.ReLU(inplace=True)
# ... 631 lines not shown
            pinned.copy_(totals, non_blocking=True)
            out.update(parts=parts, totals=pinned)
        return out

    def _forward_channels_last(self, xyz, features, new_xyz, new_xyz_feature, sampled_idx_list, prequery=None):
        B, npoint = new_xyz.shape[0], new_xyz.shape[1]
        plans = [None] * len(self.groupers)
        pending = None
        plan_parts = None
        if prequery is not None:
            idxs = prequery['idxs']
            if prequery['parts'] is not None and self.ragged_capable(features):
                plan_parts = prequery['parts']
                plans = pointnet2_utils.ragged_plans_from(prequery['parts'], prequery['totals'].tolist())
        else:
            idxs = self._ball_queries(xyz, new_xyz)
            if self.ragged_capable(features):
                parts, totals = pointnet2_utils.ragged_plan_parts(idxs)
                plan_parts = parts
                pinned = torch.empty((len(parts),), dtype=torch.int32, pin_memory=True)
                pinned.copy_(totals, non_blocking=True)
                ev = torch.cuda.Event()
                ev.record()
                if not PLAN_OVERLAP:
                    ev.synchronize()
                pending = (parts, pinned, ev)
        feats_pm = features.transpose(1, 2).contiguous()
        global_in = torch.cat([new_xyz, new_xyz_feature], dim=-1)
        centre = new_xyz.unsqueeze(2)
        pre, geo = [], []
        for i in range(len(self.groupers)):
            r, ns = self.groupers[i].radius, self.nsamples[i]
            fused_geo = (FUSED_GEOMETRY and xyz.is_cuda and xyz.dtype == torch.float32 and ns <= 64 and ns & (ns - 1) == 0
                         and not xyz.requires_grad and not new_xyz.requires_grad)
            if fused_geo:
                rppe = torch.empty((B, npoint, ns, 12), dtype=torch.float32, device=xyz.device)
                dscale = torch.empty((B, npoint, ns, 1), dtype=torch.float32, device=xyz.device)
                pointnet2_utils.pointnet2.pda_geometry(xyz.contiguous(), new_xyz.contiguous(), idxs[i], rppe, dscale,
                                                       B, xyz.shape[1], npoint, ns, r)
            else:
                nbr = pointnet2_utils.group_rows(xyz, idxs[i])
                diff = nbr - centre
                dist = torch.norm(diff, dim=-1, keepdim=True)
                density = torch.exp(-dist ** 2 / (2 * r ** 2)) / (2.5 * r)
                direction = diff / r
                dscale = density / density.max(dim=2, keepdim=True)[0]
                rppe = torch.cat([centre.expand(B, npoint, ns, 3), nbr, -diff, direction], dim=-1)
            geo.append((rppe, dscale, fused_geo))
        dns = [self.point_density[i].densitynet for i in range(len(self.groupers))]
        fused = [i for i in range(len(self.groupers)) if pointnet2_utils.DensityNetFused.supported(geo[i][1], dns[i])]
        dsc = [g[1] for g in geo]
        if fused:
            parts_f = [plan_parts[i] if (plan_parts is not None and geo[i][2]) else None for i in fused]
            for i, y in zip(fused, pointnet2_utils.densitynet_multi([dns[i] for i in fused], [dsc[i] for i in fused], parts_f)):
                dsc[i] = y
        for i in range(len(self.groupers)):
            rppe, dscale = geo[i][0], dsc[i]
            if i not in fused and _densitynet_eval_ok(dns[i], dscale):
                dscale = _densitynet_eval(dns[i], dscale)
            elif i not in fused:
                for conv, bn in zip(dns[i].mlp_convs, dns[i].mlp_bns):
                    if _can_fold(conv, bn):
                        dscale = _linear_relu(dscale, *_folded_conv_bn(conv, bn))
                    else:
                        dscale = _bn_relu_lastdim(bn, pointnet2_utils.linear(dscale, conv.weight.flatten(1), conv.bias))
            glob = _mlp_lastdim(self.global_mlps[i], global_in)
            pre.append((rppe, dscale, glob))
        if pending is not None:
            parts, pinned, ev = pending
            ev.synchronize()
            plans = pointnet2_utils.ragged_plans_from(parts, pinned.tolist())
        plans = [p if p is not None and p.fraction <= pointnet2_utils.RAGGED_MAX_FRACTION else None for p in plans]
        outs = [None] * len(self.groupers)
        order = sorted(range(len(self.groupers)), key=lambda i: -(plans[i].tokens if plans[i] is not None else npoint * self.nsamples[i] * B))
        if not PLAN_OVERLAP:
            order = list(range(len(self.groupers)))
        for i in order:
            ns = self.nsamples[i]
            rppe, dscale, glob = pre[i]
            pre[i] = None
            if (plans[i] is not None and feats_pm.shape[-1] in (16, 32, 64, 128, 256) and FUSED_BN_RELU
                    and pointnet2_utils.FUSED_ASSEMBLE and pointnet2_utils.position_mlp_ragged_supported(self.position_mlp[i], rppe)):
                rppe_c = pointnet2_utils.position_mlp_ragged(self.position_mlp[i], rppe, plans[i])
                x = pointnet2_utils.AssembleTokensRagged.apply(rppe_c, dscale, feats_pm, idxs[i], glob, plans[i])
                x = pointnet2_utils.ragged_transformer_block(self.Local_pointformer[i], x, plans[i]).view(B, npoint, -1)
                outs[i] = _mlp_lastdim(self.fin_conv[i], x)
                continue
            rppe = _mlp_lastdim(self.position_mlp[i], rppe)
            if plans[i] is not None and pointnet2_utils.AssembleTokens.supported(rppe, feats_pm):
                x = pointnet2_utils.AssembleTokensRagged.apply(rppe, dscale, feats_pm, idxs[i], glob, plans[i])
                x = pointnet2_utils.ragged_transformer_block(self.Local_pointformer[i], x, plans[i]).view(B, npoint, -1)
                outs[i] = _mlp_lastdim(self.fin_conv[i], x)
                continue
            if pointnet2_utils.AssembleTokens.supported(rppe, feats_pm):
                x = pointnet2_utils.AssembleTokens.apply(rppe, dscale, feats_pm, idxs[i], glob)
            else:
                g = pointnet2_utils.group_rows(feats_pm, idxs[i])
                x = torch.cat([rppe, g * dscale, g, glob.unsqueeze(2).expand(-1, -1, ns, -1)], dim=-1)
            D = x.shape[-1]
            x = _transformer_batch_first(self.Local_pointformer[i], x.view(B * npoint, ns, D), pool=True).view(B, npoint, D)
            outs[i] = _mlp_lastdim(self.fin_conv[i], x)
        new_features = torch.cat(outs, dim=-1)
        if self.aggregation_layer is not None:
            new_features = _mlp_lastdim(self.aggregation_layer, new_features)
        cls_features = _mlp_lastdim(self.confidence_layers, new_features) if self.confidence_layers is not None else None
        return new_xyz, new_features.transpose(1, 2).contiguous(), cls_features, sampled_idx_list


class Vote_layer(nn.Module):

    def __init__(self, mlp_list, pre_channel, max_translate_range):
        super().__init__()
        self.mlp_list = mlp_list
        if len(mlp_list) > 0:
            shared_mlps = []
            for i in range(len(mlp_list)):
                shared_mlps = [nn.Conv1d(pre_channel, mlp_list[i], kernel_size=1, bias=False),
                               nn.BatchNorm1d(mlp_list[i]), nn.ReLU()]
                pre_channel = mlp_list[i]
            self.mlp_modules = nn.Sequential(*shared_mlps)
        else:
            self.mlp_modules = None
        self.ctr_reg = nn.Conv1d(pre_channel, 3, kernel_size=1)
        self.max_offset_limit = torch.tensor(max_translate_range).float() if max_translate_range is not None else None
        self.register_buffer("_offset_limit", self.max_offset_limit.clone().view(1, 1, 3)
                             if self.max_offset_limit is not None else None, persistent=False)

    def forward(self, xyz, features):
        xyz_select = xyz
        new_features = self.mlp_modules(features) if self.mlp_modules is not None else features
        ctr_offsets = self.ctr_reg(new_features).transpose(1, 2)
        new_features = ctr_offsets[..., 3:]
        ctr_offsets = ctr_offsets[..., :3]
        if self.max_offset_limit is not None:
            lim = self._offset_limit
            limited = torch.where(ctr_offsets > lim, lim, ctr_offsets)
            limited = torch.where(limited < -lim, -lim, limited)
            vote_xyz = xyz_select + limited
        else:
            vote_xyz = xyz_select + ctr_offsets
        return vote_xyz, new_features, xyz_select, ctr_offsets


class PointnetFPModule(nn.Module):

    def __init__(self, *, mlp: List[int], bn: bool = True):
        super().__init__()
        shared_mlps = []
        for k in range(len(mlp) - 1):
            shared_mlps.extend([nn.Conv2d(mlp[k], mlp[k + 1], kernel_size=1, bias=False),
                                nn.BatchNorm2d(mlp[k + 1]), nn.ReLU()])
        self.mlp = nn.Sequential(*shared_mlps)

    def forward(self, unknown, known, unknow_feats, known_feats):
        if known is not None:
            dist, idx = pointnet2_utils.three_nn(unknown, known)
            dist_recip = 1.0 / (dist + 1e-8)
            norm = torch.sum(dist_recip, dim=2, keepdim=True)
            weight = dist_recip / norm
            interpolated_feats = pointnet2_utils.three_interpolate(known_feats, idx, weight)
        else:
            interpolated_feats = known_feats.expand(*known_feats.size()[0:2], unknown.size(1))
        if unknow_feats is not None:
            new_features = torch.cat([interpolated_feats, unknow_feats], dim=1)
        else:
            new_features = interpolated_feats
        return self.mlp(new_features.unsqueeze(-1)).squeeze(-1)
```

pdanet_amd/pointnet2_utils.py:

```python
from typing import List, Tuple

import functools
import os

import torch
import torch.nn as nn
from torch.autograd import Function

from . import _lib
from . import param_cache
from . import pointnet2_batch_cuda as pointnet2

_fwd = torch.amp.custom_fwd(device_type="cuda", cast_inputs=torch.float32)
_bwd = torch.amp.custom_bwd(device_type="cuda")


class FarthestPointSampling(Function):

    @staticmethod
    @_fwd
    def forward(ctx, xyz: torch.Tensor, npoint: int) -> torch.Tensor:
        assert xyz.is_contiguous()
        B, N, _ = xyz.size()
        output = torch.empty((B, npoint), dtype=torch.int32, device=xyz.device)
# ... 1316 lines not shown
        return out

    @staticmethod
    def backward(ctx, grad_out):
        dscale, feats_pm, idx, cnt, off, rowmap = ctx.saved_tensors
        B, N, M, ns, C, U, compact = ctx.dims
        dev = grad_out.device
        g_rppe = torch.empty((U, C) if compact else (B, M, ns, C), dtype=torch.float32, device=dev)
        g_ds = torch.empty_like(dscale)
        g_feats = torch.zeros((B, N, C), dtype=torch.float32, device=dev)
        g_glob = torch.empty((B, M, C), dtype=torch.float32, device=dev)
        pointnet2.assemble_tokens_ragged_grad(grad_out.contiguous(), dscale, feats_pm, idx, cnt, off, g_rppe, g_ds, g_feats, g_glob,
                                              U, B, N, M, ns, C, rppe_compact=compact,
                                              rowmap=rowmap if ASSEMBLE_BWD_TOKEN_PARALLEL else None)
        return g_rppe, g_ds, g_feats, None, g_glob, None


RAGGED_POSITION_MLP = True


class BatchNormReLUWeighted(Function):

    @staticmethod
    def forward(ctx, x, weight, bias, running_mean, running_var, eps, momentum, roww, count):
        x = x.contiguous()
        rows, c = x.shape
        y = torch.empty_like(x)
        stats = torch.empty((2 * c,), dtype=torch.float32, device=x.device)
        scratch = torch.empty((pointnet2.bn_relu_scratch_bytes(c),), dtype=torch.uint8, device=x.device)
        pointnet2.bn_relu_fwd_weighted(x, weight, bias, running_mean, running_var, y, stats, scratch, rows, c, eps, momentum, roww, count)
        ctx.save_for_backward(x, weight, bias, stats, roww)
        ctx.count = count
        return y

    @staticmethod
    def backward(ctx, grad_y):
        x, weight, bias, stats, roww = ctx.saved_tensors
        rows, c = x.shape
        gx = torch.empty_like(x)
        gw, gb = torch.empty_like(weight), torch.empty_like(bias)
        scratch = torch.empty((pointnet2.bn_relu_scratch_bytes(c),), dtype=torch.uint8, device=x.device)
        pointnet2.bn_relu_bwd_weighted(x, grad_y.contiguous(), weight, bias, stats, gx, gw, gb, scratch, rows, c, roww, ctx.count)
        return gx, gw, gb, None, None, None, None, None, None


def position_mlp_ragged_supported(layers, rppe):
    layers = list(layers)
    ok = (RAGGED_POSITION_MLP and rppe.is_cuda and rppe.dtype == torch.float32 and len(layers) == 6 and torch.is_grad_enabled()
          and not DENSE_BF16 and not torch.is_autocast_enabled())
    if not ok:
        return False
    for conv, bn in ((layers[0], layers[1]), (layers[3], layers[4])):
        c = conv.weight.shape[0]
        if (conv.bias is not None or not bn.training or not bn.affine or bn.momentum is None or c < 4 or c > 1024
                or (c & (c - 1)) != 0):
            return False
    return True


def position_mlp_ragged(layers, rppe, plan):
    layers = list(layers)
    x = rppe.reshape(-1, rppe.shape[-1]).index_select(0, plan.rowmap)
    count = plan.groups * plan.nsample
    for conv, bn in ((layers[0], layers[1]), (layers[3], layers[4])):
        x = linear(x, conv.weight.flatten(1), None)
        rm, rv = (bn.running_mean, bn.running_var) if bn.track_running_stats else (None, None)
        bump_bn_counter(bn)
        x = BatchNormReLUWeighted.apply(x, bn.weight, bn.bias, rm, rv, bn.eps, bn.momentum, plan.roww, count)
    return x


def _wgrad_ragged(x2d, g2d, weight, want_bias):
    n_out, n_in = weight.shape
    tokens = x2d.shape[0]
    if (LINEAR_WGRAD_KERNEL and tokens >= 4096 and (min(n_out, n_in) >= 64 or max(n_out, n_in) <= 64) and n_out % 4 == 0
            and n_in % 4 == 0 and x2d.dtype == torch.float32 and g2d.dtype == torch.float32):
        gw = torch.empty_like(weight)
        gb = torch.empty((n_out,), dtype=torch.float32, device=x2d.device) if want_bias else None
        pointnet2.linear_wgrad(x2d.contiguous(), g2d.contiguous(), gw, gb, tokens, n_in, n_out)
        return gw, gb
    return g2d.t().mm(x2d), (g2d.sum(0) if want_bias else None)


class RaggedTransformerBlock(Function):

    @staticmethod
    def supported(d, heads, nsample, x):
        return (RAGGED_TOKENS and x.is_cuda and x.dtype == torch.float32 and d in (256, 512, 1024) and d % heads == 0
                and nsample in GroupAttention.SUPPORTED_SEQ and d // heads in GroupAttention.SUPPORTED_HD
                and not torch.is_autocast_enabled() and not DENSE_BF16)

    @staticmethod
    def forward(ctx, x, plan, n1w, n1b, in_w, in_b, out_w, out_b, n2w, n2b, w1, b1, w2, b2, heads, eps1, eps2):
        x = x.contiguous()
        U, D = x.shape
        G, S, hd = plan.groups, plan.nsample, D // heads
        dev = x.device
        f32 = dict(dtype=torch.float32, device=dev)
        src1, ssum, src2 = torch.empty_like(x), torch.empty_like(x), torch.empty_like(x)
        st1, st2 = torch.empty((U, 2), **f32), torch.empty((U, 2), **f32)
        lse = torch.empty((G, heads, S), **f32)
        pointnet2.layer_norm_fwd(x, None, n1w, n1b, None, src1, st1, U, D, eps1)
        qkv = _gemm_nt(src1, in_w, in_b)
        a = torch.empty((U, D), **f32)
        pointnet2.group_attention_ragged_fwd(qkv, plan.cnt, plan.off, a, lse, U, G, S, heads, hd)
        proj = _gemm_nt(a, out_w, out_b)
        pointnet2.layer_norm_fwd(proj, src1, n2w, n2b, ssum, src2, st2, U, D, eps2)
        del proj
        h = _gemm_nt(src2, w1, b1, relu=True)
        ffn = _gemm_nt(h, w2, b2)
        y = torch.empty((G, D), **f32)
        arg = torch.empty((G, D), dtype=torch.uint8, device=dev)
        pointnet2.add_max_pool_ragged(src2, ffn, plan.cnt, plan.off, y, arg, U, G, D)
        ctx.save_for_backward(x, st1, src1, qkv, lse, a, ssum, st2, src2, h, n1w, in_w, out_w, n2w, w1, w2, arg,
                              plan.cnt, plan.off, plan.rowmap)
        ctx.heads, ctx.dims = heads, (G, S)
        return y

    @staticmethod
    @_grouped_param_grads
    def backward(ctx, dy):
        x, st1, src1, qkv, lse, a, ssum, st2, src2, h, n1w, in_w, out_w, n2w, w1, w2, arg, cnt, off, rowmap = ctx.saved_tensors
        U, D = x.shape
        G, S = ctx.dims
        heads = ctx.heads
        hd = D // heads
        dev = x.device
        f32 = dict(dtype=torch.float32, device=dev)
        dy2 = torch.empty((U, D), **f32)
        pointnet2.max_pool_scatter_ragged(dy.contiguous(), arg, rowmap, off, dy2, U, G, S, D)
        d_h = _gemm_nn(dy2, w2)
        gw2, gb2 = _wgrad_ragged(h, dy2, w2, True)
        d_h = torch.ops.aten.threshold_backward(d_h, h, 0)
        gw1, gb1 = _wgrad_ragged(src2, d_h, w1, True)
        d_lin1 = _gemm_nn(d_h, w1)
        del d_h
        d_s = torch.empty((U, D), **f32)
        gn2w, gn2b = torch.empty_like(n2w), torch.empty_like(n2w)
        scratch = torch.empty((pointnet2.layer_norm_scratch_bytes(D),), dtype=torch.uint8, device=dev)
        pointnet2.layer_norm_bwd(ssum, dy2, n2w, st2, d_s, gn2w, gn2b, scratch, U, D, grad_y2=d_lin1)
        del d_lin1
        d_a = _gemm_nn(d_s, out_w)
        gwo, gbo = _wgrad_ragged(a, d_s, out_w, True)
        dqkv = torch.empty_like(qkv)
        pointnet2.group_attention_ragged_bwd(qkv, d_a, lse, cnt, off, dqkv, U, G, S, heads, hd)
        del d_a
        gwi, gbi = _wgrad_ragged(src1, dqkv, in_w, True)
        d_src1 = _gemm_nn(dqkv, in_w, acc=d_s)
        del dqkv
        d_x = torch.empty_like(x)
        gn1w, gn1b = torch.empty_like(n1w), torch.empty_like(n1w)
        scratch1 = torch.empty_like(scratch)
        pointnet2.layer_norm_bwd(x, d_src1, n1w, st1, d_x, gn1w, gn1b, scratch1, U, D)
        return d_x, None, gn1w, gn1b, gwi, gbi, gwo, gbo, gn2w, gn2b, gw1, gb1, gw2, gb2, None, None, None


def ragged_transformer_block(tr, x, plan):
    at = tr.self_attn
    return RaggedTransformerBlock.apply(x, plan, tr.norm1.weight, tr.norm1.bias, at.in_proj_weight, at.in_proj_bias,
                                        at.out_proj.weight, at.out_proj.bias, tr.norm2.weight, tr.norm2.bias,
                                        tr.linear1.weight, tr.linear1.bias, tr.linear2.weight, tr.linear2.bias,
                                        at.num_heads, tr.norm1.eps, tr.norm2.eps)


class LayerNormResidual(Function):

    @staticmethod
    def supported(x, d):
        return x.is_cuda and x.dtype == torch.float32 and x.shape[-1] == d and d in (256, 512, 1024) and x.numel() > 0

    @staticmethod
    def forward(ctx, x, residual, weight, bias, eps):
        x = x.contiguous()
        d = x.shape[-1]
        rows = x.numel() // d
        y = torch.empty_like(x)
        stats = torch.empty((rows, 2), dtype=torch.float32, device=x.device)
        if residual is not None:
            s = torch.empty_like(x)
            pointnet2.layer_norm_fwd(x, residual.contiguous(), weight, bias, s, y, stats, rows, d, eps)
        else:
            s = x
            pointnet2.layer_norm_fwd(x, None, weight, bias, None, y, stats, rows, d, eps)
        ctx.save_for_backward(s, weight, stats)
        ctx.has_residual = residual is not None
        return y

    @staticmethod
    def backward(ctx, grad_y):
        s, weight, stats = ctx.saved_tensors
        d = s.shape[-1]
        rows = s.numel() // d
        gx = torch.empty_like(s)
        gw, gb = torch.empty_like(weight), torch.empty_like(weight)
        scratch = torch.empty((pointnet2.layer_norm_scratch_bytes(d),), dtype=torch.uint8, device=s.device)
        pointnet2.layer_norm_bwd(s, grad_y.contiguous(), weight, stats, gx, gw, gb, scratch, rows, d)
        return gx, (gx if ctx.has_residual else None), gw, gb, None


def layer_norm(x, ln, residual=None):
    return LayerNormResidual.apply(x, residual, ln.weight, ln.bias, ln.eps)


class BallQuery(Function):

    @staticmethod
    @_fwd
    def forward(ctx, radius: float, nsample: int, xyz: torch.Tensor, new_xyz: torch.Tensor) -> torch.Tensor:
        assert new_xyz.is_contiguous()
        assert xyz.is_contiguous()
        B, N, _ = xyz.size()
        npoint = new_xyz.size(1)
        idx = torch.zeros((B, npoint, nsample), dtype=torch.int32, device=xyz.device)
        pointnet2.ball_query_wrapper(B, N, npoint, radius, nsample, new_xyz, xyz, idx)
        ctx.mark_non_differentiable(idx)
        return idx

    @staticmethod
    def backward(ctx, a=None):
        return None, None, None, None


ball_query = BallQuery.apply


class BallQueryDilated(Function):

    @staticmethod
    @_fwd
    def forward(ctx, max_radius: float, min_radius: float, nsample: int, xyz: torch.Tensor,
                new_xyz: torch.Tensor) -> torch.Tensor:
        assert new_xyz.is_contiguous()
        assert xyz.is_contiguous()
        B, N, _ = xyz.size()
        npoint = new_xyz.size(1)
        idx = torch.zeros((B, npoint, nsample), dtype=torch.int32, device=xyz.device)
        pointnet2.ball_query_dilated_wrapper(B, N, npoint, max_radius, min_radius, nsample, new_xyz, xyz, idx)
        ctx.mark_non_differentiable(idx)
        return idx

    @staticmethod
    def backward(ctx, a=None):
        return None, None, None, None, None


# ... 148 lines not shown
```

Baseline: 124.9 scenes/s.

## Fuse ragged token assembly with first LayerNorm, add pooled BN backward sums

Token assembly (rppe, density scale, gathered features, global feature) is fused into the first LayerNorm of the ragged transformer block in forward and backward. The assembled token tensor is never materialized, which removes a full write and re-read of the U×D activation and one kernel launch per direction. Separately, the BN+ReLU+maxpool backward gets a reduction kernel that iterates only over pooled groups and gathers the argmax rows instead of scanning every row. Both paths are on by default behind env toggles, and they add more complex gather-and-scatter gradient code.

```diff
diff --git a/include/pda_train.h b/include/pda_train.h
--- a/include/pda_train.h
+++ b/include/pda_train.h
@@ -144,6 +144,17 @@
                                     float *grad_rppe, float *grad_dscale, float *grad_feats, float *grad_glob,
                                     int64_t max_tokens, int b, int n, int m, int nsample, int c, int rppe_compact,
                                     pda_stream_t stream);
+int pda_assemble_ln_ragged_fwd(const float *rppe, const float *dscale, const float *feats, const int32_t *idx,
+                               const float *glob, const int32_t *rowmap, const float *gamma, const float *beta,
+                               float *src1, float *mean_rstd, int64_t tokens, int b, int n, int m, int nsample, int c,
+                               int rppe_compact, float eps, pda_stream_t stream);
+int pda_assemble_ln_ragged_bwd_partials(const float *grad_src1, const float *mean_rstd, const float *rppe,
+                                        const float *dscale, const float *feats, const int32_t *idx, const float *glob,
+                                        const int32_t *rowmap, const int32_t *cnt, const int32_t *off,
+                                        const float *gamma, float *grad_rppe, float *grad_dscale, float *grad_feats,
+                                        float *grad_glob, float *grad_glob_tokens, void *ln_scratch, int64_t tokens,
+                                        int b, int n, int m, int nsample, int c, int rppe_compact, int *nblocks,
+                                        pda_stream_t stream);
 int pda_add_max_pool_ragged(const float *a, const float *b, const int32_t *cnt, const int32_t *off, float *out,
                             uint8_t *arg, int64_t groups, int d, pda_stream_t stream);
 int pda_max_pool_scatter_ragged(const float *grad_out, const uint8_t *arg, const int32_t *rowmap,
diff --git a/pdanet_amd/_lib.py b/pdanet_amd/_lib.py
--- a/pdanet_amd/_lib.py
+++ b/pdanet_amd/_lib.py
@@ -122,6 +122,8 @@
     "pda_ragged_plan": [_vp, _vp, _vp, _vp, _vp, ctypes.c_int64, _i, _vp],
     "pda_assemble_tokens_ragged": [_vp, _vp, _vp, _vp, _vp, _vp, _vp, _vp, ctypes.c_int64, _i, _i, _i, _i, _i, _i, _vp],
     "pda_assemble_tokens_ragged_grad": [_vp, _vp, _vp, _vp, _vp, _vp, _vp, _vp, _vp, _vp, _vp, ctypes.c_int64, _i, _i, _i, _i, _i, _i, _vp],
+    "pda_assemble_ln_ragged_fwd": [_vp] * 10 + [ctypes.c_int64, _i, _i, _i, _i, _i, _i, _f, _vp],
+    "pda_assemble_ln_ragged_bwd_partials": [_vp] * 17 + [ctypes.c_int64, _i, _i, _i, _i, _i, _i, ctypes.POINTER(_i), _vp],
     "pda_bn_relu_fwd_weighted": [_vp, _vp, _vp, _vp, _vp, _vp, _vp, _vp, ctypes.c_int64, _i, _f, _f, _vp, ctypes.c_int64, _vp],
     "pda_bn_relu_bwd_weighted": [_vp, _vp, _vp, _vp, _vp, _vp, _vp, _vp, _vp, ctypes.c_int64, _i, _vp, ctypes.c_int64, _vp],
     "pda_add_max_pool_ragged": [_vp, _vp, _vp, _vp, _vp, _vp, ctypes.c_int64, _i, _vp],
diff --git a/pdanet_amd/csrc/bn_relu.hip b/pdanet_amd/csrc/bn_relu.hip
--- a/pdanet_amd/csrc/bn_relu.hip
+++ b/pdanet_amd/csrc/bn_relu.hip
@@ -93,6 +93,42 @@
     block_reduce_cols(a, b, lds, s.cg, s.rpb, pa, pa + s.c);
 }
 
+template <typename TX>
+__global__ __launch_bounds__(256) void bn_pool_sums_kernel(const TX* __restrict__ x, const float* __restrict__ gout,
+                                                           const uint8_t* __restrict__ arg, const float* __restrict__ mean_invstd,
+                                                           const float* __restrict__ gamma, const float* __restrict__ beta,
+                                                           double* __restrict__ partial, int64_t groups, BnShape s) {
+    __shared__ double lds[2 * 256 * 4];
+    const int tid = threadIdx.x;
+    const int col = tid % s.cg, r0 = tid / s.cg;
+    const float4 mu = reinterpret_cast<const float4*>(mean_invstd)[col], is = reinterpret_cast<const float4*>(mean_invstd + s.c)[col];
+    const float4 g = reinterpret_cast<const float4*>(gamma)[col], be = reinterpret_cast<const float4*>(beta)[col];
+    const float muv[4] = {mu.x, mu.y, mu.z, mu.w}, isv[4] = {is.x, is.y, is.z, is.w}, gg[4] = {g.x, g.y, g.z, g.w},
+                bb[4] = {be.x, be.y, be.z, be.w};
+    double a[4] = {0, 0, 0, 0}, b[4] = {0, 0, 0, 0};
+    const int64_t stride = (int64_t)gridDim.x * s.rpb;
+#pragma unroll 2
+    for (int64_t q = (int64_t)blockIdx.x * s.rpb + r0; q < groups; q += stride) {
+        const float4 d = reinterpret_cast<const float4*>(gout)[q * s.cg + col];
+        const uchar4 k = reinterpret_cast<const uchar4*>(arg)[q * s.cg + col];
+        const int kk[4] = {k.x, k.y, k.z, k.w};
+        const float dd[4] = {d.x, d.y, d.z, d.w};
+        const TX* px = x + (size_t)q * s.ns * s.c + 4 * col;
+        float v[4];
+#pragma unroll
+        for (int j = 0; j < 4; ++j) v[j] = kk[j] < s.ns ? load1(px + (size_t)kk[j] * s.c + j) : 0.f;
+#pragma unroll
+        for (int j = 0; j < 4; ++j) {
+            const float xh = (v[j] - muv[j]) * isv[j];
+            const float dyh = (kk[j] < s.ns && xh * gg[j] + bb[j] > 0.f) ? dd[j] : 0.f;
+            a[j] += dyh;
+            b[j] += (double)dyh * xh;
+        }
+    }
+    double* pa = partial + (size_t)blockIdx.x * 2 * s.c;
+    block_reduce_cols(a, b, lds, s.cg, s.rpb, pa, pa + s.c);
+}
+
 __device__ __forceinline__ bool sum_partials(const double* __restrict__ partial, int nblocks, int c, double& s1, double& s2, int& ch) {
     __shared__ double red[2][16][32];
     const int cl = threadIdx.x & 31, part = threadIdx.x >> 5;
@@ -326,9 +362,18 @@
                     ((uintptr_t)arg & 3) == 0, "%s: alignment", what);
     const int grid = bn_grid(s);
     float* sums = reinterpret_cast<float*>(reinterpret_cast<double*>(scratch) + (size_t)BN_BLOCKS * 2 * c);
-    hipLaunchKernelGGL((bn_reduce_kernel<true, TX, float, true>), dim3(grid), dim3(256), 0, st, x, grad_out, mean_invstd, gamma, beta,
-                       (double*)scratch, s, arg);
-    hipLaunchKernelGGL(bn_finalize_bwd_kernel, dim3(divup(c, 32)), dim3(512), 0, st, (const double*)scratch, grid, c, s.rows, grad_gamma, grad_beta,
+    const char* e = getenv("PDA_BN_POOL_SUMS");
+    int nparts = grid;
+    if (!e || atoi(e) != 0) {
+        const int64_t steps = divup64(groups, s.rpb);
+        nparts = (int)(steps < BN_BLOCKS ? steps : BN_BLOCKS);
+        hipLaunchKernelGGL(bn_pool_sums_kernel<TX>, dim3(nparts), dim3(256), 0, st, x, grad_out, arg, mean_invstd, gamma, beta, (double*)scratch,
+                           groups, s);
+    } else {
+        hipLaunchKernelGGL((bn_reduce_kernel<true, TX, float, true>), dim3(grid), dim3(256), 0, st, x, grad_out, mean_invstd, gamma, beta,
+                           (double*)scratch, s, arg);
+    }
+    hipLaunchKernelGGL(bn_finalize_bwd_kernel, dim3(divup(c, 32)), dim3(512), 0, st, (const double*)scratch, nparts, c, s.rows, grad_gamma, grad_beta,
                        sums);
     hipLaunchKernelGGL((bn_apply_kernel<true, TX, float, TX, true>), dim3(grid), dim3(256), 0, st, x, grad_out, mean_invstd, gamma, beta, sums,
                        grad_x, s, arg);
diff --git a/pdanet_amd/csrc/layer_norm.hip b/pdanet_amd/csrc/layer_norm.hip
--- a/pdanet_amd/csrc/layer_norm.hip
+++ b/pdanet_amd/csrc/layer_norm.hip
@@ -1,15 +1,8 @@
 #include "pda_common.h"
+#include "layer_norm_row.h"
 #include "param_grad_reduce.h"
 
 namespace pda {
-
-constexpr int LN_BLOCKS = 1024;
-
-__device__ __forceinline__ float wave_sum(float v) {
-#pragma unroll
-    for (int o = 32; o >= 1; o >>= 1) v += __shfl_xor(v, o);
-    return v;
-}
 
 template <int V, bool RESIDUAL, typename TX>
 __global__ __launch_bounds__(256) void layer_norm_fwd_kernel(const TX* __restrict__ x, const float* __restrict__ res,
@@ -26,8 +19,7 @@
         be[v] = reinterpret_cast<const float4*>(beta)[v * 64 + lane];
     }
     for (int64_t r = (int64_t)blockIdx.x * 4 + wave_id(); r < rows; r += (int64_t)gridDim.x * 4) {
-        float4 a[V];
-        float s = 0.f;
+        float4 a[V], o[V];
 #pragma unroll
         for (int v = 0; v < V; ++v) {
             a[v] = load4(x + r * D + 4 * (v * 64 + lane));
@@ -36,25 +28,13 @@
                 a[v].x += b.x; a[v].y += b.y; a[v].z += b.z; a[v].w += b.w;
                 reinterpret_cast<float4*>(sum_out + r * D)[v * 64 + lane] = a[v];
             }
-            s += (a[v].x + a[v].y) + (a[v].z + a[v].w);
-        }
-        const float mean = wave_sum(s) * (1.0f / D);
-        float q = 0.f;
-#pragma unroll
-        for (int v = 0; v < V; ++v) {
-            const float dx = a[v].x - mean, dy = a[v].y - mean, dz = a[v].z - mean, dw = a[v].w - mean;
-            q += (dx * dx + dy * dy) + (dz * dz + dw * dw);
-        }
-        const float rstd = 1.0f / sqrtf(wave_sum(q) * (1.0f / D) + eps);
-#pragma unroll
-        for (int v = 0; v < V; ++v) {
-            float4 o;
-            o.x = (a[v].x - mean) * rstd * g[v].x + be[v].x;
-            o.y = (a[v].y - mean) * rstd * g[v].y + be[v].y;
-            o.z = (a[v].z - mean) * rstd * g[v].z + be[v].z;
-            o.w = (a[v].w - mean) * rstd * g[v].w + be[v].w;
-            if (y) reinterpret_cast<float4*>(y + r * D)[v * 64 + lane] = o;
-            if (yb) store4(yb + r * D + 4 * (v * 64 + lane), o);
+        }
+        float mean, rstd;
+        ln_row_fwd<V>(a, g, be, eps, o, mean, rstd);
+#pragma unroll
+        for (int v = 0; v < V; ++v) {
+            if (y) reinterpret_cast<float4*>(y + r * D)[v * 64 + lane] = o[v];
+            if (yb) store4(yb + r * D + 4 * (v * 64 + lane), o[v]);
         }
         if (lane == 0) { mean_rstd[r * 2] = mean; mean_rstd[r * 2 + 1] = rstd; }
     }
@@ -76,56 +56,30 @@
     }
     for (int64_t r = (int64_t)blockIdx.x * 4 + w; r < rows; r += (int64_t)gridDim.x * 4) {
         const float mean = mean_rstd[r * 2], rstd = mean_rstd[r * 2 + 1];
-        float4 xh[V], d[V];
-        float s1 = 0.f, s2 = 0.f;
-#pragma unroll
-        for (int v = 0; v < V; ++v) {
-            const float4 xv = reinterpret_cast<const float4*>(x + r * D)[v * 64 + lane];
+        float4 xv[V], d[V], o[V];
+#pragma unroll
+        for (int v = 0; v < V; ++v) {
+            xv[v] = reinterpret_cast<const float4*>(x + r * D)[v * 64 + lane];
             d[v] = reinterpret_cast<const float4*>(dy + r * D)[v * 64 + lane];
             if (TWO) {
                 const float4 e = load4(dy2 + r * D + 4 * (v * 64 + lane));
                 d[v].x += e.x; d[v].y += e.y; d[v].z += e.z; d[v].w += e.w;
             }
-            xh[v] = make_float4((xv.x - mean) * rstd, (xv.y - mean) * rstd, (xv.z - mean) * rstd, (xv.w - mean) * rstd);
-            sb[v].x += d[v].x; sb[v].y += d[v].y; sb[v].z += d[v].z; sb[v].w += d[v].w;
-            sg[v].x += d[v].x * xh[v].x; sg[v].y += d[v].y * xh[v].y; sg[v].z += d[v].z * xh[v].z; sg[v].w += d[v].w * xh[v].w;
-            d[v].x *= g[v].x; d[v].y *= g[v].y; d[v].z *= g[v].z; d[v].w *= g[v].w;
-            s1 += (d[v].x + d[v].y) + (d[v].z + d[v].w);
-            s2 += (d[v].x * xh[v].x + d[v].y * xh[v].y) + (d[v].z * xh[v].z + d[v].w * xh[v].w);
-        }
-        const float m1 = wave_sum(s1) * (1.0f / D), m2 = wave_sum(s2) * (1.0f / D);
-#pragma unroll
-        for (int v = 0; v < V; ++v) {
-            float4 o;
-            o.x = rstd * (d[v].x - m1 - xh[v].x * m2);
-            o.y = rstd * (d[v].y - m1 - xh[v].y * m2);
-            o.z = rstd * (d[v].z - m1 - xh[v].z * m2);
-            o.w = rstd * (d[v].w - m1 - xh[v].w * m2);
-            reinterpret_cast<float4*>(dx + r * D)[v * 64 + lane] = o;
-            if (dxb) store4(dxb + r * D + 4 * (v * 64 + lane), o);
-        }
-    }
-#pragma unroll
-    for (int v = 0; v < V; ++v) {
-        reinterpret_cast<float4*>(red[0][w])[v * 64 + lane] = sb[v];
-        reinterpret_cast<float4*>(red[1][w])[v * 64 + lane] = sg[v];
-    }
-    __syncthreads();
-    for (int c = threadIdx.x; c < D; c += 256) {
-        partial[((size_t)blockIdx.x * 2 + 0) * D + c] = (red[0][0][c] + red[0][1][c]) + (red[0][2][c] + red[0][3][c]);
-        partial[((size_t)blockIdx.x * 2 + 1) * D + c] = (red[1][0][c] + red[1][1][c]) + (red[1][2][c] + red[1][3][c]);
-    }
+        }
+        ln_row_bwd<V>(xv, d, g, mean, rstd, sb, sg, o);
+#pragma unroll
+        for (int v = 0; v < V; ++v) {
+            reinterpret_cast<float4*>(dx + r * D)[v * 64 + lane] = o[v];
+            if (dxb) store4(dxb + r * D + 4 * (v * 64 + lane), o[v]);
+        }
+    }
+    ln_write_partials<V>(sb, sg, red, partial);
 }
 
 __global__ __launch_bounds__(1024) void layer_norm_finalize_kernel(const float* __restrict__ partial, int nblocks, int d,
                                                                    float* __restrict__ dgamma, float* __restrict__ dbeta) {
     __shared__ float red[2][16][64];
     layer_norm_finalize_block(partial, nblocks, d, dgamma, dbeta, (int)blockIdx.x, red);
-}
-
-static int ln_grid(int64_t rows) {
-    const int64_t b = divup64(rows, 4);
-    return (int)(b < LN_BLOCKS ? b : LN_BLOCKS);
 }
 
 }
diff --git a/pdanet_amd/csrc/layer_norm_row.h b/pdanet_amd/csrc/layer_norm_row.h
--- /dev/null
+++ b/pdanet_amd/csrc/layer_norm_row.h
@@ -0,0 +1,85 @@
+#pragma once
+#include "pda_common.h"
+
+namespace pda {
+
+constexpr int LN_BLOCKS = 1024;
+
+static inline int ln_grid(int64_t rows) {
+    const int64_t b = divup64(rows, 4);
+    return (int)(b < LN_BLOCKS ? b : LN_BLOCKS);
+}
+
+__device__ __forceinline__ float wave_sum(float v) {
+#pragma unroll
+    for (int o = 32; o >= 1; o >>= 1) v += __shfl_xor(v, o);
+    return v;
+}
+
+template <int V>
+__device__ __forceinline__ void ln_row_fwd(const float4 (&a)[V], const float4 (&g)[V], const float4 (&be)[V], float eps,
+                                           float4 (&o)[V], float& mean, float& rstd) {
+    constexpr int D = 256 * V;
+    float s = 0.f;
+#pragma unroll
+    for (int v = 0; v < V; ++v) s += (a[v].x + a[v].y) + (a[v].z + a[v].w);
+    mean = wave_sum(s) * (1.0f / D);
+    float q = 0.f;
+#pragma unroll
+    for (int v = 0; v < V; ++v) {
+        const float dx = a[v].x - mean, dy = a[v].y - mean, dz = a[v].z - mean, dw = a[v].w - mean;
+        q += (dx * dx + dy * dy) + (dz * dz + dw * dw);
+    }
+    rstd = 1.0f / sqrtf(wave_sum(q) * (1.0f / D) + eps);
+#pragma unroll
+    for (int v = 0; v < V; ++v) {
+        o[v].x = (a[v].x - mean) * rstd * g[v].x + be[v].x;
+        o[v].y = (a[v].y - mean) * rstd * g[v].y + be[v].y;
+        o[v].z = (a[v].z - mean) * rstd * g[v].z + be[v].z;
+        o[v].w = (a[v].w - mean) * rstd * g[v].w + be[v].w;
+    }
+}
+
+template <int V>
+__device__ __forceinline__ void ln_row_bwd(const float4 (&xv)[V], float4 (&d)[V], const float4 (&g)[V], float mean, float rstd,
+                                           float4 (&sb)[V], float4 (&sg)[V], float4 (&o)[V]) {
+    constexpr int D = 256 * V;
+    float4 xh[V];
+    float s1 = 0.f, s2 = 0.f;
+#pragma unroll
+    for (int v = 0; v < V; ++v) {
+        xh[v] = make_float4((xv[v].x - mean) * rstd, (xv[v].y - mean) * rstd, (xv[v].z - mean) * rstd, (xv[v].w - mean) * rstd);
+        sb[v].x += d[v].x; sb[v].y += d[v].y; sb[v].z += d[v].z; sb[v].w += d[v].w;
+        sg[v].x += d[v].x * xh[v].x; sg[v].y += d[v].y * xh[v].y; sg[v].z += d[v].z * xh[v].z; sg[v].w += d[v].w * xh[v].w;
+        d[v].x *= g[v].x; d[v].y *= g[v].y; d[v].z *= g[v].z; d[v].w *= g[v].w;
+        s1 += (d[v].x + d[v].y) + (d[v].z + d[v].w);
+        s2 += (d[v].x * xh[v].x + d[v].y * xh[v].y) + (d[v].z * xh[v].z + d[v].w * xh[v].w);
+    }
+    const float m1 = wave_sum(s1) * (1.0f / D), m2 = wave_sum(s2) * (1.0f / D);
+#pragma unroll
+    for (int v = 0; v < V; ++v) {
+        o[v].x = rstd * (d[v].x - m1 - xh[v].x * m2);
+        o[v].y = rstd * (d[v].y - m1 - xh[v].y * m2);
+        o[v].z = rstd * (d[v].z - m1 - xh[v].z * m2);
+        o[v].w = rstd * (d[v].w - m1 - xh[v].w * m2);
+    }
+}
+
+template <int V>
+__device__ __forceinline__ void ln_write_partials(const float4 (&sb)[V], const float4 (&sg)[V], float (&red)[2][4][256 * V],
+                                                  float* __restrict__ partial) {
+    constexpr int D = 256 * V;
+    const int lane = lane_id(), w = wave_id();
+#pragma unroll
+    for (int v = 0; v < V; ++v) {
+        reinterpret_cast<float4*>(red[0][w])[v * 64 + lane] = sb[v];
+        reinterpret_cast<float4*>(red[1][w])[v * 64 + lane] = sg[v];
+    }
+    __syncthreads();
+    for (int c = threadIdx.x; c < D; c += 256) {
+        partial[((size_t)blockIdx.x * 2 + 0) * D + c] = (red[0][0][c] + red[0][1][c]) + (red[0][2][c] + red[0][3][c]);
+        partial[((size_t)blockIdx.x * 2 + 1) * D + c] = (red[1][0][c] + red[1][1][c]) + (red[1][2][c] + red[1][3][c]);
+    }
+}
+
+}
diff --git a/pdanet_amd/csrc/ragged.hip b/pdanet_amd/csrc/ragged.hip
--- a/pdanet_amd/csrc/ragged.hip
+++ b/pdanet_amd/csrc/ragged.hip
@@ -1,4 +1,5 @@
 #include "pda_common.h"
+#include "layer_norm_row.h"
 
 namespace pda {
 
@@ -149,7 +150,8 @@
     atomicAdd(df + 2, g_fd.z * d + g_f.z); atomicAdd(df + 3, g_fd.w * d + g_f.w);
 }
 
-__global__ __launch_bounds__(256) void assemble_ragged_bwd_group_kernel(const float* __restrict__ dx, const int32_t* __restrict__ cnt,
+__global__ __launch_bounds__(256) void assemble_ragged_bwd_group_kernel(const float* __restrict__ gglob, int64_t stride4,
+                                                                        const int32_t* __restrict__ cnt,
                                                                         const int32_t* __restrict__ off, float* __restrict__ d_rppe,
                                                                         float* __restrict__ d_dscale, float* __restrict__ d_glob, int c4,
                                                                         int ns, int64_t total, int rppe_compact) {
@@ -158,23 +160,137 @@
     const int c = (int)(e % c4);
     const int64_t bm = e / c4;
     const int n_tok = cnt[bm];
-    const float4* g4 = reinterpret_cast<const float4*>(dx) + (size_t)off[bm] * 4 * c4 + 3 * c4 + c;
+    const float4* g4 = reinterpret_cast<const float4*>(gglob) + (size_t)off[bm] * stride4 + c;
     float4 acc = make_float4(0.f, 0.f, 0.f, 0.f);
     int t = 0;
     for (; t + 4 <= n_tok; t += 4) {
         float4 v[4];
 #pragma unroll
-        for (int q = 0; q < 4; ++q) v[q] = g4[(size_t)(t + q) * 4 * c4];
+        for (int q = 0; q < 4; ++q) v[q] = g4[(size_t)(t + q) * stride4];
 #pragma unroll
         for (int q = 0; q < 4; ++q) { acc.x += v[q].x; acc.y += v[q].y; acc.z += v[q].z; acc.w += v[q].w; }
     }
-    for (; t < n_tok; ++t) { const float4 v = g4[(size_t)t * 4 * c4]; acc.x += v.x; acc.y += v.y; acc.z += v.z; acc.w += v.w; }
+    for (; t < n_tok; ++t) { const float4 v = g4[(size_t)t * stride4]; acc.x += v.x; acc.y += v.y; acc.z += v.z; acc.w += v.w; }
     reinterpret_cast<float4*>(d_glob)[bm * c4 + c] = acc;
     const float4 zero = make_float4(0.f, 0.f, 0.f, 0.f);
     for (t = n_tok; t < ns; ++t) {
         if (!rppe_compact) reinterpret_cast<float4*>(d_rppe)[(size_t)(bm * ns + t) * c4 + c] = zero;
         if (c == 0) d_dscale[bm * ns + t] = 0.f;
     }
+}
+
+
+template <int V>
+__device__ __forceinline__ void assemble_row(const float* __restrict__ rppe_row, const float* __restrict__ feat_row,
+                                             const float* __restrict__ glob_row, float d, int lane, float4 (&a)[V], float4 (&f)[V]) {
+    constexpr int c4 = 16 * V;
+#pragma unroll
+    for (int v = 0; v < V; ++v) {
+        const int j = v * 64 + lane, q = j / c4, c = j % c4;
+        const float* p = q == 0 ? rppe_row : (q == 3 ? glob_row : feat_row);
+        f[v] = reinterpret_cast<const float4*>(p)[c];
+        a[v] = q == 1 ? make_float4(f[v].x * d, f[v].y * d, f[v].z * d, f[v].w * d) : f[v];
+    }
+}
+
+template <int V>
+__global__ __launch_bounds__(256) void assemble_ln_ragged_fwd_kernel(const float* __restrict__ rppe, const float* __restrict__ dscale,
+                                                                     const float* __restrict__ feats, const int* __restrict__ idx,
+                                                                     const float* __restrict__ glob, const int32_t* __restrict__ rowmap,
+                                                                     const float* __restrict__ gamma, const float* __restrict__ beta,
+                                                                     float* __restrict__ y, float* __restrict__ mean_rstd, int64_t rows,
+                                                                     int n, int m, int ns, int64_t slots, int rppe_compact, float eps) {
+    constexpr int D = 256 * V, C = 64 * V;
+    const int lane = lane_id();
+    float4 g[V], be[V];
+#pragma unroll
+    for (int v = 0; v < V; ++v) {
+        g[v] = reinterpret_cast<const float4*>(gamma)[v * 64 + lane];
+        be[v] = reinterpret_cast<const float4*>(beta)[v * 64 + lane];
+    }
+    for (int64_t r = (int64_t)blockIdx.x * 4 + wave_id(); r < rows; r += (int64_t)gridDim.x * 4) {
+        const int64_t tok = __builtin_amdgcn_readfirstlane(rowmap[r]);
+        if (tok < 0 || tok >= slots) continue;
+        const int row = __builtin_amdgcn_readfirstlane(idx[tok]);
+        if (row < 0 || row >= n) continue;
+        const int64_t bm = tok / ns, b = bm / m;
+        float4 a[V], f[V], o[V];
+        assemble_row<V>(rppe + (size_t)(rppe_compact ? r : tok) * C, feats + ((size_t)b * n + row) * C, glob + (size_t)bm * C, dscale[tok],
+                        lane, a, f);
+        float mean, rstd;
+        ln_row_fwd<V>(a, g, be, eps, o, mean, rstd);
+#pragma unroll
+        for (int v = 0; v < V; ++v) reinterpret_cast<float4*>(y + r * D)[v * 64 + lane] = o[v];
+        if (lane == 0) { mean_rstd[r * 2] = mean; mean_rstd[r * 2 + 1] = rstd; }
+    }
+}
+
+template <int V>
+__global__ __launch_bounds__(256) void assemble_ln_ragged_bwd_kernel(const float* __restrict__ dy, const float* __restrict__ mean_rstd,
+                                                                     const float* __restrict__ rppe, const float* __restrict__ dscale,
+                                                                     const float* __restrict__ feats, const int* __restrict__ idx,
+                                                                     const float* __restrict__ glob, const int32_t* __restrict__ rowmap,
+                                                                     const float* __restrict__ gamma, float* __restrict__ d_rppe,
+                                                                     float* __restrict__ d_dscale, float* __restrict__ d_feats,
+                                                                     float* __restrict__ g_glob, float* __restrict__ partial, int64_t rows,
+                                                                     int n, int m, int ns, int64_t slots, int rppe_compact) {
+    static_assert(V == 1 || V == 2, "the f * d and f quarters share a chunk index (V = 1) or a lane range (V = 2)");
+    constexpr int D = 256 * V, C = 64 * V, c4 = 16 * V;
+    __shared__ float red[2][4][D];
+    const int lane = lane_id();
+    float4 g[V], sb[V], sg[V];
+#pragma unroll
+    for (int v = 0; v < V; ++v) {
+        g[v] = reinterpret_cast<const float4*>(gamma)[v * 64 + lane];
+        sb[v] = make_float4(0, 0, 0, 0); sg[v] = make_float4(0, 0, 0, 0);
+    }
+    for (int64_t r = (int64_t)blockIdx.x * 4 + wave_id(); r < rows; r += (int64_t)gridDim.x * 4) {
+        const int64_t tok = __builtin_amdgcn_readfirstlane(rowmap[r]);
+        if (tok < 0 || tok >= slots) continue;
+        const int row = __builtin_amdgcn_readfirstlane(idx[tok]);
+        if (row < 0 || row >= n) continue;
+        const int64_t bm = tok / ns, b = bm / m;
+        const float mean = mean_rstd[r * 2], rstd = mean_rstd[r * 2 + 1];
+        const float ds = dscale[tok];
+        float4 xv[V], f[V], d[V], o[V];
+        assemble_row<V>(rppe + (size_t)(rppe_compact ? r : tok) * C, feats + ((size_t)b * n + row) * C, glob + (size_t)bm * C, ds, lane, xv, f);
+#pragma unroll
+        for (int v = 0; v < V; ++v) d[v] = reinterpret_cast<const float4*>(dy + r * D)[v * 64 + lane];
+        ln_row_bwd<V>(xv, d, g, mean, rstd, sb, sg, o);
+#pragma unroll
+        for (int v = 0; v < V; ++v) {
+            const int j = v * 64 + lane, q = j / c4, c = j % c4;
+            if (q == 0) reinterpret_cast<float4*>(d_rppe + (size_t)(rppe_compact ? r : tok) * C)[c] = o[v];
+            if (q == 3) reinterpret_cast<float4*>(g_glob + (size_t)r * C)[c] = o[v];
+        }
+        const bool fd_lane = lane >= c4 && lane < 2 * c4;
+        float part = fd_lane ? (o[0].x * f[0].x + o[0].y * f[0].y) + (o[0].z * f[0].z + o[0].w * f[0].w) : 0.f;
+#pragma unroll
+        for (int s = c4 >> 1; s >= 1; s >>= 1) part += __shfl_xor(part, s);
+        if (lane == c4) d_dscale[tok] = part;
+        float4 val;
+        int base;
+        if constexpr (V == 1) {
+            const int src = (lane + 16) & 63;
+            val = make_float4(o[0].x * ds + __shfl(o[0].x, src), o[0].y * ds + __shfl(o[0].y, src), o[0].z * ds + __shfl(o[0].z, src),
+                              o[0].w * ds + __shfl(o[0].w, src));
+            base = 16;
+        } else {
+            const int src = (lane + 32) & 63;
+            val = make_float4(__shfl(o[0].x, src) * ds + o[1].x, __shfl(o[0].y, src) * ds + o[1].y, __shfl(o[0].z, src) * ds + o[1].z,
+                              __shfl(o[0].w, src) * ds + o[1].w);
+            base = 0;
+        }
+        float* df = d_feats + ((size_t)b * n + row) * C;
+#pragma unroll
+        for (int i = 0; i < V; ++i) {
+            const int src = base + i * 16 + (lane >> 2);
+            const float t0 = __shfl(val.x, src), t1 = __shfl(val.y, src), t2 = __shfl(val.z, src), t3 = __shfl(val.w, src);
+            const int k = lane & 3;
+            atomicAdd(df + i * 64 + lane, k == 0 ? t0 : (k == 1 ? t1 : (k == 2 ? t2 : t3)));
+        }
+    }
+    ln_write_partials<V>(sb, sg, red, partial);
 }
 
 __global__ __launch_bounds__(256) void add_max_pool_ragged_kernel(const float* __restrict__ a, const float* __restrict__ b,
@@ -277,8 +393,8 @@
             switch (c / 4) { PDA_ASM_TOK(4); PDA_ASM_TOK(8); PDA_ASM_TOK(16); PDA_ASM_TOK(32); PDA_ASM_TOK(64); }
 #undef PDA_ASM_TOK
         }
-        hipLaunchKernelGGL(pda::assemble_ragged_bwd_group_kernel, grid, block, 0, (hipStream_t)stream, grad_out, cnt, off, grad_rppe,
-                           grad_dscale, grad_glob, c / 4, nsample, centre_cols, rppe_compact);
+        hipLaunchKernelGGL(pda::assemble_ragged_bwd_group_kernel, grid, block, 0, (hipStream_t)stream, grad_out + 3 * c, (int64_t)c, cnt, off,
+                           grad_rppe, grad_dscale, grad_glob, c / 4, nsample, centre_cols, rppe_compact);
         return pda::check_launch("pda_assemble_tokens_ragged_grad");
     }
 #define PDA_ASM_BWD(C4)                                                                                                          \
@@ -287,6 +403,67 @@
     switch (c / 4) { PDA_ASM_BWD(4); PDA_ASM_BWD(8); PDA_ASM_BWD(16); PDA_ASM_BWD(32); PDA_ASM_BWD(64); }
 #undef PDA_ASM_BWD
     return pda::check_launch("pda_assemble_tokens_ragged_grad");
+}
+
+static int assemble_ln_sizes(const char* what, int64_t tokens, int b, int n, int m, int nsample, int c) {
+    PDA_REQUIRE(tokens >= 0 && b >= 0 && n >= 1 && m >= 0 && nsample >= 1 && (c == 64 || c == 128) &&
+                    (int64_t)b * m * nsample < INT32_MAX && tokens <= (int64_t)b * m * nsample,
+                "%s: bad size: tokens=%lld b=%d n=%d m=%d nsample=%d C=%d (64 or 128)", what, (long long)tokens, b, n, m, nsample, c);
+    return PDA_OK;
+}
+
+PDA_API int pda_assemble_ln_ragged_fwd(const float* rppe, const float* dscale, const float* feats, const int32_t* idx, const float* glob,
+                                       const int32_t* rowmap, const float* gamma, const float* beta, float* src1, float* mean_rstd,
+                                       int64_t tokens, int b, int n, int m, int nsample, int c, int rppe_compact, float eps,
+                                       pda_stream_t stream) {
+    if (int rc = assemble_ln_sizes("pda_assemble_ln_ragged_fwd", tokens, b, n, m, nsample, c)) return rc;
+    if (tokens == 0) return PDA_OK;
+    PDA_REQUIRE(rppe && dscale && feats && idx && glob && rowmap && gamma && beta && src1 && mean_rstd,
+                "pda_assemble_ln_ragged_fwd: null pointer");
+    PDA_REQUIRE((((uintptr_t)rppe | (uintptr_t)feats | (uintptr_t)glob | (uintptr_t)gamma | (uintptr_t)beta | (uintptr_t)src1) & 15) == 0,
+                "pda_assemble_ln_ragged_fwd: alignment");
+    const dim3 grid(pda::ln_grid(tokens)), block(256);
+    const int64_t slots = (int64_t)b * m * nsample;
+    if (c == 64)
+        hipLaunchKernelGGL(pda::assemble_ln_ragged_fwd_kernel<1>, grid, block, 0, (hipStream_t)stream, rppe, dscale, feats, idx, glob, rowmap,
+                           gamma, beta, src1, mean_rstd, tokens, n, m, nsample, slots, rppe_compact, eps);
+    else
+        hipLaunchKernelGGL(pda::assemble_ln_ragged_fwd_kernel<2>, grid, block, 0, (hipStream_t)stream, rppe, dscale, feats, idx, glob, rowmap,
+                           gamma, beta, src1, mean_rstd, tokens, n, m, nsample, slots, rppe_compact, eps);
+    return pda::check_launch("pda_assemble_ln_ragged_fwd");
+}
+
+PDA_API int pda_assemble_ln_ragged_bwd_partials(const float* grad_src1, const float* mean_rstd, const float* rppe, const float* dscale,
+                                                const float* feats, const int32_t* idx, const float* glob, const int32_t* rowmap,
+                                                const int32_t* cnt, const int32_t* off, const float* gamma, float* grad_rppe,
+                                                float* grad_dscale, float* grad_feats, float* grad_glob, float* grad_glob_tokens,
+                                                void* ln_scratch, int64_t tokens, int b, int n, int m, int nsample, int c,
+                                                int rppe_compact, int* nblocks, pda_stream_t stream) {
+    if (int rc = assemble_ln_sizes("pda_assemble_ln_ragged_bwd_partials", tokens, b, n, m, nsample, c)) return rc;
+    PDA_REQUIRE(tokens >= 1 && (int64_t)b * m >= 1, "pda_assemble_ln_ragged_bwd_partials: bad size: tokens=%lld b=%d m=%d", (long long)tokens, b, m);
+    PDA_REQUIRE(grad_src1 && mean_rstd && rppe && dscale && feats && idx && glob && rowmap && cnt && off && gamma && grad_rppe && grad_dscale &&
+                    grad_feats && grad_glob && grad_glob_tokens && ln_scratch && nblocks,
+                "pda_assemble_ln_ragged_bwd_partials: null pointer");
+    PDA_REQUIRE((((uintptr_t)grad_src1 | (uintptr_t)rppe | (uintptr_t)feats | (uintptr_t)glob | (uintptr_t)gamma | (uintptr_t)grad_rppe |
+                  (uintptr_t)grad_glob | (uintptr_t)grad_glob_tokens) & 15) == 0,
+                "pda_assemble_ln_ragged_bwd_partials: alignment");
+    const int nb = pda::ln_grid(tokens);
+    const dim3 grid(nb), block(256);
+    const int64_t slots = (int64_t)b * m * nsample;
+    if (c == 64)
+        hipLaunchKernelGGL(pda::assemble_ln_ragged_bwd_kernel<1>, grid, block, 0, (hipStream_t)stream, grad_src1, mean_rstd, rppe, dscale, feats,
+                           idx, glob, rowmap, gamma, grad_rppe, grad_dscale, grad_feats, grad_glob_tokens, (float*)ln_scratch, tokens, n, m,
+                           nsample, slots, rppe_compact);
+    else
+        hipLaunchKernelGGL(pda::assemble_ln_ragged_bwd_kernel<2>, grid, block, 0, (hipStream_t)stream, grad_src1, mean_rstd, rppe, dscale, feats,
+                           idx, glob, rowmap, gamma, grad_rppe, grad_dscale, grad_feats, grad_glob_tokens, (float*)ln_scratch, tokens, n, m,
+                           nsample, slots, rppe_compact);
+    const int64_t centre_cols = (int64_t)b * m * (c / 4);
+    hipLaunchKernelGGL(pda::assemble_ragged_bwd_group_kernel, dim3((unsigned)pda::divup64(centre_cols, 256)), block, 0, (hipStream_t)stream,
+                       (const float*)grad_glob_tokens, (int64_t)(c / 4), cnt, off, grad_rppe, grad_dscale, grad_glob, c / 4, nsample, centre_cols,
+                       rppe_compact);
+    *nblocks = nb;
+    return pda::check_launch("pda_assemble_ln_ragged_bwd_partials");
 }
 
 PDA_API int pda_add_max_pool_ragged(const float* a, const float* b, const int32_t* cnt, const int32_t* off, float* out, uint8_t* arg,
diff --git a/pdanet_amd/pointnet2_batch_cuda.py b/pdanet_amd/pointnet2_batch_cuda.py
--- a/pdanet_amd/pointnet2_batch_cuda.py
+++ b/pdanet_amd/pointnet2_batch_cuda.py
@@ -768,6 +768,45 @@
     return 1
 
 
+def assemble_ln_ragged_fwd(rppe, dscale, feats, idx, glob, rowmap, gamma, beta, src1, mean_rstd, tokens, b, n, m, nsample, c, eps,
+                           rppe_compact=False):
+    t = b * m * nsample
+    _numel_ok(rppe, (tokens if rppe_compact else t) * c, "rppe"); _numel_ok(dscale, t, "dscale"); _numel_ok(feats, b * n * c, "feats"); _numel_ok(idx, t, "idx")
+    _numel_ok(glob, b * m * c, "glob"); _numel_ok(rowmap, tokens, "rowmap"); _numel_ok(gamma, 4 * c, "gamma"); _numel_ok(beta, 4 * c, "beta")
+    _numel_ok(src1, tokens * 4 * c, "src1"); _numel_ok(mean_rstd, tokens * 2, "mean_rstd")
+    _call("pda_assemble_ln_ragged_fwd", rppe, _chk(rppe, "rppe", F32), _chk(dscale, "dscale", F32), _chk(feats, "feats", F32),
+          _chk(idx, "idx", I32), _chk(glob, "glob", F32), _chk(rowmap, "rowmap", I32), _chk(gamma, "gamma", F32), _chk(beta, "beta", F32),
+          _chk(src1, "src1", F32), _chk(mean_rstd, "mean_rstd", F32), tokens, b, n, m, nsample, c, 1 if rppe_compact else 0, float(eps))
+    return 1
+
+
+def assemble_ln_ragged_bwd(grad_src1, mean_rstd, rppe, dscale, feats, idx, glob, rowmap, cnt, off, gamma, grad_rppe, grad_dscale, grad_feats,
+                           grad_glob, grad_gamma, grad_beta, scratch, tokens, b, n, m, nsample, c, rppe_compact=False):
+    t = b * m * nsample
+    _numel_ok(grad_src1, tokens * 4 * c, "grad_src1"); _numel_ok(mean_rstd, tokens * 2, "mean_rstd")
+    _numel_ok(rppe, (tokens if rppe_compact else t) * c, "rppe"); _numel_ok(dscale, t, "dscale"); _numel_ok(feats, b * n * c, "feats"); _numel_ok(idx, t, "idx")
+    _numel_ok(glob, b * m * c, "glob"); _numel_ok(rowmap, tokens, "rowmap"); _numel_ok(cnt, b * m, "cnt"); _numel_ok(off, b * m + 1, "off")
+    _numel_ok(gamma, 4 * c, "gamma"); _numel_ok(grad_rppe, (tokens if rppe_compact else t) * c, "grad_rppe"); _numel_ok(grad_dscale, t, "grad_dscale")
+    _numel_ok(grad_feats, b * n * c, "grad_feats"); _numel_ok(grad_glob, b * m * c, "grad_glob")
+    _numel_ok(grad_gamma, 4 * c, "grad_gamma"); _numel_ok(grad_beta, 4 * c, "grad_beta"); _numel_ok(scratch, layer_norm_scratch_bytes(4 * c), "scratch")
+    glob_tokens = torch.empty((tokens, c), dtype=F32, device=grad_src1.device)
+    nblocks = ctypes.c_int(0)
+    _call("pda_assemble_ln_ragged_bwd_partials", grad_src1, _chk(grad_src1, "grad_src1", F32), _chk(mean_rstd, "mean_rstd", F32),
+          _chk(rppe, "rppe", F32), _chk(dscale, "dscale", F32), _chk(feats, "feats", F32), _chk(idx, "idx", I32), _chk(glob, "glob", F32),
+          _chk(rowmap, "rowmap", I32), _chk(cnt, "cnt", I32), _chk(off, "off", I32), _chk(gamma, "gamma", F32),
+          _chk(grad_rppe, "grad_rppe", F32), _chk(grad_dscale, "grad_dscale", F32), _chk(grad_feats, "grad_feats", F32),
+          _chk(grad_glob, "grad_glob", F32), _chk(glob_tokens, "grad_glob_tokens", F32), _chk(scratch, "scratch", torch.uint8),
+          tokens, b, n, m, nsample, c, 1 if rppe_compact else 0, ctypes.byref(nblocks))
+    entry = _lib.ParamGradEntry(1, nblocks.value, scratch.data_ptr(), None, _chk(grad_gamma, "grad_gamma", F32),
+                                _chk(grad_beta, "grad_beta", F32), 0, 4 * c, 0, 0)
+    group = _open_group()
+    if group is not None:
+        group.add(entry, scratch, grad_gamma, grad_beta)
+    else:
+        _call("pda_param_grad_reduce_grouped", scratch, (_lib.ParamGradEntry * 1)(entry), 1)
+    return 1
+
+
 def add_max_pool_ragged(a, b, cnt, off, out, arg, tokens, groups, d):
     _numel_ok(a, tokens * d, "a"); _numel_ok(b, tokens * d, "b"); _numel_ok(out, groups * d, "out"); _numel_ok(arg, groups * d, "arg")
     _numel_ok(cnt, groups, "cnt"); _numel_ok(off, groups + 1, "off")
diff --git a/pdanet_amd/pointnet2_modules.py b/pdanet_amd/pointnet2_modules.py
--- a/pdanet_amd/pointnet2_modules.py
+++ b/pdanet_amd/pointnet2_modules.py
@@ -737,14 +737,14 @@
             if (plans[i] is not None and feats_pm.shape[-1] in (16, 32, 64, 128, 256) and FUSED_BN_RELU
                     and pointnet2_utils.FUSED_ASSEMBLE and pointnet2_utils.position_mlp_ragged_supported(self.position_mlp[i], rppe)):
                 rppe_c = pointnet2_utils.position_mlp_ragged(self.position_mlp[i], rppe, plans[i])
-                x = pointnet2_utils.AssembleTokensRagged.apply(rppe_c, dscale, feats_pm, idxs[i], glob, plans[i])
-                x = pointnet2_utils.ragged_transformer_block(self.Local_pointformer[i], x, plans[i]).view(B, npoint, -1)
+                x = pointnet2_utils.assemble_and_ragged_transformer_block(self.Local_pointformer[i], rppe_c, dscale, feats_pm, idxs[i], glob,
+                                                                          plans[i]).view(B, npoint, -1)
                 outs[i] = _mlp_lastdim(self.fin_conv[i], x)
                 continue
             rppe = _mlp_lastdim(self.position_mlp[i], rppe)
             if plans[i] is not None and pointnet2_utils.AssembleTokens.supported(rppe, feats_pm):
-                x = pointnet2_utils.AssembleTokensRagged.apply(rppe, dscale, feats_pm, idxs[i], glob, plans[i])
-                x = pointnet2_utils.ragged_transformer_block(self.Local_pointformer[i], x, plans[i]).view(B, npoint, -1)
+                x = pointnet2_utils.assemble_and_ragged_transformer_block(self.Local_pointformer[i], rppe, dscale, feats_pm, idxs[i], glob,
+                                                                          plans[i]).view(B, npoint, -1)
                 outs[i] = _mlp_lastdim(self.fin_conv[i], x)
                 continue
             if pointnet2_utils.AssembleTokens.supported(rppe, feats_pm):
diff --git a/pdanet_amd/pointnet2_utils.py b/pdanet_amd/pointnet2_utils.py
--- a/pdanet_amd/pointnet2_utils.py
+++ b/pdanet_amd/pointnet2_utils.py
@@ -1422,6 +1422,9 @@
     return g2d.t().mm(x2d), (g2d.sum(0) if want_bias else None)
 
 
+ASSEMBLE_LN_FUSED = os.environ.get("PDA_ASSEMBLE_LN_FUSED", "1") != "0"
+
+
 class RaggedTransformerBlock(Function):
 
     @staticmethod
@@ -1431,16 +1434,33 @@
                 and not torch.is_autocast_enabled() and not DENSE_BF16)
 
     @staticmethod
-    def forward(ctx, x, plan, n1w, n1b, in_w, in_b, out_w, out_b, n2w, n2b, w1, b1, w2, b2, heads, eps1, eps2):
-        x = x.contiguous()
-        U, D = x.shape
+    def fused_front(d, feats_pm):
+        return ASSEMBLE_LN_FUSED and d in (256, 512) and feats_pm.shape[-1] * 4 == d
+
+    @staticmethod
+    def forward(ctx, x, plan, n1w, n1b, in_w, in_b, out_w, out_b, n2w, n2b, w1, b1, w2, b2, heads, eps1, eps2,
+                rppe=None, dscale=None, feats_pm=None, idx=None, glob=None):
+        fused = x is None
+        if fused:
+            B, M, ns = idx.shape
+            C, N = feats_pm.shape[-1], feats_pm.shape[1]
+            rppe, dscale, feats_pm, glob = rppe.contiguous(), dscale.contiguous(), feats_pm.contiguous(), glob.contiguous()
+            U, D = plan.tokens, 4 * C
+            dev = rppe.device
+        else:
+            x = x.contiguous()
+            U, D = x.shape
+            dev = x.device
         G, S, hd = plan.groups, plan.nsample, D // heads
-        dev = x.device
         f32 = dict(dtype=torch.float32, device=dev)
-        src1, ssum, src2 = torch.empty_like(x), torch.empty_like(x), torch.empty_like(x)
+        src1, ssum, src2 = torch.empty((U, D), **f32), torch.empty((U, D), **f32), torch.empty((U, D), **f32)
         st1, st2 = torch.empty((U, 2), **f32), torch.empty((U, 2), **f32)
         lse = torch.empty((G, heads, S), **f32)
-        pointnet2.layer_norm_fwd(x, None, n1w, n1b, None, src1, st1, U, D, eps1)
+        if fused:
+            pointnet2.assemble_ln_ragged_fwd(rppe, dscale, feats_pm, idx, glob, plan.rowmap, n1w, n1b, src1, st1, U, B, N, M, ns, C, eps1,
+                                             rppe_compact=rppe.dim() == 2)
+        else:
+            pointnet2.layer_norm_fwd(x, None, n1w, n1b, None, src1, st1, U, D, eps1)
         qkv = _gemm_nt(src1, in_w, in_b)
         a = torch.empty((U, D), **f32)
         pointnet2.group_attention_ragged_fwd(qkv, plan.cnt, plan.off, a, lse, U, G, S, heads, hd)
@@ -1452,20 +1472,21 @@
         y = torch.empty((G, D), **f32)
         arg = torch.empty((G, D), dtype=torch.uint8, device=dev)
         pointnet2.add_max_pool_ragged(src2, ffn, plan.cnt, plan.off, y, arg, U, G, D)
-        ctx.save_for_backward(x, st1, src1, qkv, lse, a, ssum, st2, src2, h, n1w, in_w, out_w, n2w, w1, w2, arg,
-                              plan.cnt, plan.off, plan.rowmap)
+        front = (rppe, dscale, feats_pm, idx, glob) if fused else (x,)
+        ctx.save_for_backward(st1, src1, qkv, lse, a, ssum, st2, src2, h, n1w, in_w, out_w, n2w, w1, w2, arg,
+                              plan.cnt, plan.off, plan.rowmap, *front)
         ctx.heads, ctx.dims = heads, (G, S)
         return y
 
     @staticmethod
     @_grouped_param_grads
     def backward(ctx, dy):
-        x, st1, src1, qkv, lse, a, ssum, st2, src2, h, n1w, in_w, out_w, n2w, w1, w2, arg, cnt, off, rowmap = ctx.saved_tensors
-        U, D = x.shape
+        st1, src1, qkv, lse, a, ssum, st2, src2, h, n1w, in_w, out_w, n2w, w1, w2, arg, cnt, off, rowmap, *front = ctx.saved_tensors
+        U, D = src1.shape
         G, S = ctx.dims
         heads = ctx.heads
         hd = D // heads
-        dev = x.device
+        dev = src1.device
         f32 = dict(dtype=torch.float32, device=dev)
         dy2 = torch.empty((U, D), **f32)
         pointnet2.max_pool_scatter_ragged(dy.contiguous(), arg, rowmap, off, dy2, U, G, S, D)
@@ -1488,19 +1509,41 @@
         gwi, gbi = _wgrad_ragged(src1, dqkv, in_w, True)
         d_src1 = _gemm_nn(dqkv, in_w, acc=d_s)
         del dqkv
-        d_x = torch.empty_like(x)
         gn1w, gn1b = torch.empty_like(n1w), torch.empty_like(n1w)
         scratch1 = torch.empty_like(scratch)
-        pointnet2.layer_norm_bwd(x, d_src1, n1w, st1, d_x, gn1w, gn1b, scratch1, U, D)
-        return d_x, None, gn1w, gn1b, gwi, gbi, gwo, gbo, gn2w, gn2b, gw1, gb1, gw2, gb2, None, None, None
-
-
-def ragged_transformer_block(tr, x, plan):
+        if len(front) == 1:
+            x, = front
+            d_x = torch.empty_like(x)
+            pointnet2.layer_norm_bwd(x, d_src1, n1w, st1, d_x, gn1w, gn1b, scratch1, U, D)
+            return d_x, None, gn1w, gn1b, gwi, gbi, gwo, gbo, gn2w, gn2b, gw1, gb1, gw2, gb2, None, None, None
+        rppe, dscale, feats_pm, idx, glob = front
+        B, M, ns = idx.shape
+        C, N = feats_pm.shape[-1], feats_pm.shape[1]
+        g_rppe = torch.empty_like(rppe)
+        g_ds = torch.empty_like(dscale)
+        g_feats = torch.zeros((B, N, C), **f32)
+        g_glob = torch.empty((B, M, C), **f32)
+        pointnet2.assemble_ln_ragged_bwd(d_src1, st1, rppe, dscale, feats_pm, idx, glob, rowmap, cnt, off, n1w, g_rppe, g_ds, g_feats, g_glob,
+                                         gn1w, gn1b, scratch1, U, B, N, M, ns, C, rppe_compact=rppe.dim() == 2)
+        return (None, None, gn1w, gn1b, gwi, gbi, gwo, gbo, gn2w, gn2b, gw1, gb1, gw2, gb2, None, None, None,
+                g_rppe, g_ds, g_feats, None, g_glob)
+
+
+def ragged_transformer_block(tr, x, plan, sources=None):
     at = tr.self_attn
-    return RaggedTransformerBlock.apply(x, plan, tr.norm1.weight, tr.norm1.bias, at.in_proj_weight, at.in_proj_bias,
-                                        at.out_proj.weight, at.out_proj.bias, tr.norm2.weight, tr.norm2.bias,
-                                        tr.linear1.weight, tr.linear1.bias, tr.linear2.weight, tr.linear2.bias,
-                                        at.num_heads, tr.norm1.eps, tr.norm2.eps)
+    args = (plan, tr.norm1.weight, tr.norm1.bias, at.in_proj_weight, at.in_proj_bias,
+            at.out_proj.weight, at.out_proj.bias, tr.norm2.weight, tr.norm2.bias,
+            tr.linear1.weight, tr.linear1.bias, tr.linear2.weight, tr.linear2.bias,
+            at.num_heads, tr.norm1.eps, tr.norm2.eps)
+    if sources is not None:
+        return RaggedTransformerBlock.apply(None, *args, *sources)
+    return RaggedTransformerBlock.apply(x, *args)
+
+
+def assemble_and_ragged_transformer_block(tr, rppe, dscale, feats_pm, idx, glob, plan):
+    if RaggedTransformerBlock.fused_front(tr.self_attn.embed_dim, feats_pm):
+        return ragged_transformer_block(tr, None, plan, sources=(rppe, dscale, feats_pm, idx, glob))
+    return ragged_transformer_block(tr, AssembleTokensRagged.apply(rppe, dscale, feats_pm, idx, glob, plan), plan)
 
 
 class LayerNormResidual(Function):
```

Measured after the change: 126.5 scenes/s (median of 6 runs). No clear change (+1.3%).
